# datvo06/MSAU

Measured on AMD Instinct MI355X. Metric: chargrid tiles/sec (train fwd+bwd), 336x256x64 3-stage MSAU, higher is better.
Workload: dtype bf16; 1 GPU; configs[1]: one-hot chargrid 336x256x64, 3-stage MSAU (featRoot 8, 4 scales, res_depth 2), batch 16/GPU, fwd+masked-CE+bwd+clip+Adam; global_batch=16, parallelism=dp1, graph=False

## Files before the change

include/msau_hip.h:

```cpp
#ifndef MSAU_HIP_H
#define MSAU_HIP_H

#include <stdint.h>

#ifdef __cplusplus
extern "C" {
#endif

typedef enum { MSAU_F32 = 0, MSAU_BF16 = 1 } msau_dtype;

typedef enum {
    MSAU_OK = 0,
    MSAU_ERR_ARG = -1,
    MSAU_ERR_LDS = -2,
    MSAU_ERR_HIP = -3
} msau_status;

const char* msau_last_error(void);
int msau_version(void);
const char* msau_source_hash(void);
int msau_sizeof(int which);
int msau_lds_pixel_stride(int raw_bytes, int esz, int c8_per_chunk, int read_stride);
int msau_lds_wrow_stride(int nks, int esz);

enum {
    MSAU_CONV_RELU_IN  = 1,
    MSAU_CONV_RELU_OUT = 2,
    MSAU_CONV_ADD      = 4,
    MSAU_CONV_ACCUM    = 8,
    MSAU_CONV_MASK_A   = 16,
    MSAU_CONV_MASK_B   = 32,
    MSAU_CONV_DOUT     = 128,
    MSAU_CONV_LRN      = 256,
    MSAU_CONV_POOL     = 512,
    MSAU_CONV_IDS      = 1024,
    MSAU_CONV_OWNER    = 2048,
    MSAU_CONV_NCHW     = 4096,
    MSAU_CONV_WGRAD    = 8192,
    MSAU_CONV_ELU      = 32768,
    MSAU_CONV_EXTENT   = 65536,
    MSAU_CONV_HEAD     = 64
};

typedef struct {
    int32_t B, Hin, Win, Hout, Wout;
    int32_t C1, C2;
    int32_t Cout;
    int32_t KH, KW, dil;
    int32_t pad_t, pad_l;
    int32_t stride;
    int32_t ups;
    int32_t flags;
    const void* x1;
    const void* x2;
    const void* wpack;
    const float* bias;
    const void* add;
    const void* mask_a;
    const void* mask_b;
    void* y;
    float* head_probs;
    uint8_t* head_argmax;
    int32_t head_classes;
    int32_t flags2;
    void* y2;
    const void* mask_b2;
    float lrn_alpha_over_n, lrn_beta, lrn_k;
    int32_t reserved0;
    void* pool_y;
    uint8_t* pool_idx;
    const void* wg_x1;
    float* wg_slabs;
    int32_t wg_nslabs;
    int32_t reserved1;
    const int32_t* extent;
} msau_conv_desc;
int msau_conv2d_rider_slabs(int dtype, const msau_conv_desc* d);

typedef struct {
    int32_t cch;
    int32_t nchunks;
    int32_t kchunk;
    int32_t rows;
    int64_t bytes;
} msau_conv_pack_geom;

int msau_conv_pack_geometry(int dtype, int C1_stored, int C2_stored, int Cout_stored, int KH, int KW, int dil,
                            int stride, int ups, msau_conv_pack_geom* out);
int msau_conv2d(void* stream, int dtype, const msau_conv_desc* d);
int msau_conv2d_launch_info(int dtype, const msau_conv_desc* d, int32_t* info8);

enum { MSAU_PAIR_RELU_IN = 1, MSAU_PAIR_RELU_MID = 2, MSAU_PAIR_MASK_MID = 4,
       MSAU_PAIR_LRN_BWD = 16,
       MSAU_PAIR_WGRAD1 = 32,
       MSAU_PAIR_COUPLE = 64,
       MSAU_PAIR_DCOUPLE = 128,
       MSAU_PAIR_TILES = 8 };
typedef struct {
    int32_t B, H, W, C;
    int32_t flags1, flags2;
    const void* x;
    const void* w1;
    const float* b1;
    const void* mask_mid;
    void* mid;
    const void* w2;
    const float* b2;
    const void* add;
    const void* mask_a;
    const void* mask_b;
    void* y;
    void* pool_y;
    uint8_t* pool_idx;
    uint8_t* bits_mid;
    uint8_t* bits_a;
    const void* lrn_a;
    void* lrn_da;
    float lrn_alpha_over_n, lrn_beta, lrn_k;
    int32_t reserved0;
    const void* wg1_x;
    float* wg1_slabs;
    int32_t wg1_nslabs;
    int32_t reserved1;
    const void* cpl_prev;
    const void* cpl_w;
    const float* cpl_b;
    void* cpl_y;
    void* cpl_pool_y;
    uint8_t* cpl_pool_idx;
    const void* dcp_dz;
    const void* dcp_w;
    const void* dcp_mask;
    void* dcp_dprev;
} msau_conv_pair_desc;
int msau_conv_pair_applicable(int dtype, const msau_conv_pair_desc* d);
int msau_conv_pair(void* stream, int dtype, const msau_conv_pair_desc* d);
int64_t msau_conv_pair_bits_bytes(int dtype, const msau_conv_pair_desc* d);
int msau_conv_pair_wgrad_slabs(int dtype, const msau_conv_pair_desc* d);
int msau_conv_pair_instance(int dtype, const msau_conv_pair_desc* d);
void msau_reload_env(void);

typedef struct {
    int32_t B, Hin, Win, Hout, Wout;
    int32_t C1, C2, Cout;
    int32_t KH, KW, dil, pad_t, pad_l, stride;
    int32_t flags;
    const void* x1;
    const void* x2;
    const void* g;
    float* slabs;
    int32_t nslabs;
} msau_wgrad_desc;

typedef struct {
    int32_t cch, nchunks;
    int32_t kext;
    int32_t max_slabs;
    int64_t slab_bytes;
    int32_t lean;
    int32_t reserved;
} msau_wgrad_geom;

int msau_wgrad_geometry(int dtype, const msau_wgrad_desc* d, msau_wgrad_geom* out);
int msau_conv2d_wgrad(void* stream, int dtype, const msau_wgrad_desc* d);
int msau_conv2d_wgrad_groupable(int dtype, const msau_wgrad_desc* a, const msau_wgrad_desc* b);
int msau_conv2d_wgrad_group(void* stream, int dtype, const msau_wgrad_desc* const* ds, int n);

typedef struct {
    int64_t src_off;
    int64_t dst_off;
    int32_t kind;
    int32_t dim0, dim1;
    int32_t KH, KW;
// ... 69 lines not shown
    const void* add;
    const void* mask_b;
    void* dx;
    int64_t npix;
    int32_t C, accumulate;
} msau_attn_proj_bwd_args;
int msau_attn_proj_bwd(void* stream, int dtype, const msau_attn_proj_bwd_args* a);

typedef struct {
    const void* g;
    const void* w1_pack; const void* w2_pack;
    void* dx1; void* dx2;
    const void* mask1; const void* mask2;
    int64_t npix;
    int32_t C, accumulate1, accumulate2, reserved;
} msau_dgrad2_args;
int msau_dgrad2_1x1(void* stream, int dtype, const msau_dgrad2_args* a);

int msau_label_counts(void* stream, const int64_t* labels, int32_t* counts, int B, int64_t hw);
int msau_label_counts_split(void* stream, const int64_t* labels, int32_t* partial, int B, int64_t hw, int K);
int64_t msau_ce_ws_floats(int64_t npix_total);
int msau_masked_ce(void* stream, int dtype, const void* logits, const int64_t* labels, const int32_t* counts,
                   void* dlogits, float* loss_accum, float* ws, int B, int64_t hw, int C, int Cs, float scale);
int64_t msau_ce_multi_ws_floats(int64_t npix_total);
int msau_masked_ce_multi(void* stream, int dtype, const void* logits, const void* aux, const int64_t* labels,
                         const int32_t* counts, void* dlogits, void* daux, float* loss, float* ws,
                         int B, int64_t hw, int C, int Cs, float scale, int counts_k);

int msau_softmax_ce(void* stream, int dtype, const void* logits, const int64_t* labels, void* dlogits,
                    float* loss_accum, float* ws, int B, int64_t hw, int C, int Cs, float scale);
int msau_softmax_ce_weighted(void* stream, int dtype, const void* logits, const int64_t* labels, const float* class_w,
                             void* dlogits, float* sums, float* ws, int B, int64_t hw, int C, int Cs);

int64_t msau_adam_ws_floats(int64_t n);
int msau_clip_adam_step(void* stream, float* params, const float* grads, float* m, float* v, float* state,
                        float* ws, int64_t n, float lr, float beta1, float beta2, float eps, float max_norm,
                        float grad_scale);

int msau_raster_owner(void* stream, const int32_t* boxes, int n, int32_t* owner, int B, int H, int W);
int msau_raster_onehot(void* stream, int dtype, const int32_t* boxes, const int32_t* owner, void* grid_nhwc,
                       int B, int H, int W, int C, int Cs);
int msau_raster_labels(void* stream, const int32_t* boxes, const int32_t* owner, int64_t* labels, int B, int H, int W);
int msau_raster_dense(void* stream, int dtype, const int32_t* boxes, const int32_t* owner, const float* feats,
                      void* grid_nhwc, int B, int H, int W, int C, int Cs);

int64_t msau_box_integral_ws_floats(int B, int H, int W, int C);
int msau_box_integral(void* stream, int dtype, const void* in_nhwc, float* ii, float* ws, int B, int H, int W, int C, int Cs, int relu_in);
int msau_box_params(void* stream, const float* flat_params, int64_t off_hmin, int64_t off_hmax, int64_t off_wmin, int64_t off_wmax,
                    int C, int F, float max_h, float max_w, float* params_fwd, float* params_refl);
int msau_box_filter(void* stream, int dtype, const float* ii, const float* params, void* out_nhwc, int B, int H, int W, int C, int F,
                    int Cs_out, int sum_filters, int accumulate, const void* mask_a, const void* add, const void* mask_b);
int64_t msau_box_pgrad_ws_floats(int B, int H, int W, int C, int F);
int msau_box_param_grad(void* stream, int dtype, const float* ii, const float* params, const void* gout_nhwc, float* ws, float* flat_grads,
                        int64_t off_hmin, int64_t off_hmax, int64_t off_wmin, int64_t off_wmax, int B, int H, int W, int C, int F,
                        int Cs_out, float max_h, float max_w);

typedef struct {
    const void* in; float* ii; const float* params_fwd; const float* params_refl; void* out;
    const void* gout; void* gin; float* ii_g; float* ws; float* flat_grads; float* ws_ii;
    const void* mask_a; const void* add; const void* mask_b;
    int64_t off_hmin, off_hmax, off_wmin, off_wmax;
    int32_t B, H, W, C, F, Cs_in, Cs_out, relu_in, accumulate;
    float max_h, max_w;
} msau_box_args;
int msau_box_fwd(void* stream, int dtype, const msau_box_args* a);
int msau_box_bwd(void* stream, int dtype, const msau_box_args* a);

enum {
    MSAU_OP_CONV2D = 1,
    MSAU_OP_WGRAD = 2,
    MSAU_OP_LRN_FWD = 3,
    MSAU_OP_LRN_BWD = 4,
    MSAU_OP_POOL_FWD = 5,
    MSAU_OP_POOL_BWD = 6,
    MSAU_OP_ATTN_FWD = 7,
    MSAU_OP_ATTN_BWD = 8,
    MSAU_OP_CHANNEL_SUM = 9,
    MSAU_OP_WGRAD_REDUCE = 10,
    MSAU_OP_CONV_PAIR = 11,
    MSAU_OP_BOX_FWD = 12,
    MSAU_OP_BOX_BWD = 13,
    MSAU_OP_ALLREDUCE = 14,
    MSAU_OP_ATTN_PROJ_BWD = 15,
    MSAU_OP_DGRAD2_1X1 = 16
};
typedef struct { int32_t kind; int32_t dtype; const void* args; } msau_op;
typedef struct { const void* a; const void* dy; void* out; int64_t npix; int32_t C, Cs, n; float alpha, beta, k; } msau_lrn_args;
typedef struct { const void* x_or_dy; void* y_or_dx; uint8_t* idx; const void* mask; int32_t B, H, W, Cs, accumulate;
                 const int32_t* extent; } msau_pool_args;
typedef struct { const void* f; const void* g; const void* h; const void* x_or_dy; void* y; float* stats;
                 void* df; void* dg; void* dh; float* ws; int32_t B, N, Ds, Cs; const int32_t* extent; int32_t W, reserved0; } msau_attn_args;
typedef struct { const void* g; int64_t npix; int32_t Cs; float* partials; int32_t nblk; } msau_csum_args;
typedef struct { const float* slab_arena; float* flat_grads; const msau_unpack_entry* table_dev; int32_t n_entries, max_elems; } msau_reduce_args;
typedef struct { void* comm; float* buf; int64_t count; } msau_allreduce_args;
int msau_run_ops(void* stream, const msau_op* ops, int n);
#define MSAU_OP_SIDE 0x100
int msau_run_ops_overlap(void* stream, void* side_stream, const msau_op* ops, int n, int join);
#define MSAU_OP_JOIN 0x800
#define MSAU_OP_PROBE 0x200
#define MSAU_OP_COMM 0x400
int msau_run_ops_dp(void* stream, void* side_stream, void* comm_stream, const msau_op* ops, int n, int join);
int msau_probe_read(float* us, int cap, int* n);
int msau_probe_overhead(void* stream, int reps, float* us);

int msau_comm_available(void);
int msau_comm_unique_id(void* id128_out, int bytes);
int msau_comm_init(void** comm_out, int world, int rank, const void* id128, int bytes);
int msau_comm_destroy(void* comm);
int msau_allreduce_bucket(void* stream, void* comm, float* buf, int64_t count);

typedef struct {
    const int32_t* owner;
    const int32_t* boxes;
    const float* feats;
    const float* w;
    float* wt;
    float* table;
    float* sums;
    float* csum;
    int32_t n_boxes, n_vec, C, csum_blocks;
    int32_t wt_floats;
    int32_t reserved0;
} msau_owner_ctx;

int msau_owner_slabs(const msau_wgrad_desc* d);

int msau_spin(void* stream, int microseconds);
int msau_fill_zero(void* stream, void* p, int64_t bytes);
int msau_fork_visibility_check(void* stream, void* side_stream, int iters, int64_t words, int system_fence, int64_t* mismatches);
int msau_stream_create(int priority, void** stream_out);
int msau_stream_destroy(void* stream);
int msau_softmax_channels_nchw(void* stream, const float* logits, float* pred, int B, int C, int64_t hw);

int msau_softmax_argmax_nhwc(void* stream, int dtype, const void* logits, float* probs, uint8_t* argmax,
                             int64_t npix, int C, int Cs);
int msau_onehot_ids(void* stream, int dtype, const int32_t* ids, void* grid_nhwc, int64_t npix, int C, int Cs);
int msau_onehot_ids_ext(void* stream, int dtype, const int32_t* ids, void* grid_nhwc, int B, int H, int W, int C, int Cs,
                        const int32_t* extent);
int msau_eval_confusion(void* stream, int dtype, const void* logits, const int64_t* labels, int64_t* counts, int B, int H, int W,
                        int C, int Cs, int zero_as, const int32_t* extent);

#ifdef __cplusplus
}
#endif
#endif
```

msau_amd/_lib.py:

```python
from __future__ import annotations

import ctypes as C
import os

HERE = os.path.dirname(os.path.abspath(__file__))
LIB_PATH = os.environ.get("MSAU_HIP_LIB", os.path.join(HERE, "libmsau_hip.so"))

F32, BF16 = 0, 1

CONV_RELU_IN, CONV_RELU_OUT, CONV_ADD, CONV_ACCUM, CONV_MASK_A, CONV_MASK_B, CONV_HEAD, CONV_DOUT = 1, 2, 4, 8, 16, 32, 64, 128
CONV_LRN, CONV_POOL, CONV_IDS, CONV_OWNER, CONV_NCHW, CONV_WGRAD, CONV_ELU = 256, 512, 1024, 2048, 4096, 8192, 32768
CONV_EXTENT = 65536

i32, i64, vp, f32 = C.c_int32, C.c_int64, C.c_void_p, C.c_float


class ConvDesc(C.Structure):
    _fields_ = [(n, i32) for n in ("B", "Hin", "Win", "Hout", "Wout", "C1", "C2", "Cout", "KH", "KW", "dil",
                                   "pad_t", "pad_l", "stride", "ups", "flags")] + \
               [(n, vp) for n in ("x1", "x2", "wpack", "bias", "add", "mask_a", "mask_b", "y", "head_probs", "head_argmax")] + \
               [("head_classes", i32), ("flags2", i32), ("y2", vp), ("mask_b2", vp)] + \
               [("lrn_alpha_over_n", f32), ("lrn_beta", f32), ("lrn_k", f32), ("reserved0", i32), ("pool_y", vp), ("pool_idx", vp)] + \
               [("wg_x1", vp), ("wg_slabs", vp), ("wg_nslabs", i32), ("reserved1", i32), ("extent", vp)]

# ... 10 lines not shown


class BoxArgs(C.Structure):
    _fields_ = [(n, vp) for n in ("in_", "ii", "params_fwd", "params_refl", "out", "gout", "gin", "ii_g", "ws", "flat_grads", "ws_ii",
                                  "mask_a", "add", "mask_b")] + \
               [(n, i64) for n in ("off_hmin", "off_hmax", "off_wmin", "off_wmax")] + \
               [(n, i32) for n in ("B", "H", "W", "C", "F", "Cs_in", "Cs_out", "relu_in", "accumulate")] + \
               [("max_h", f32), ("max_w", f32)]


class ConvPackGeom(C.Structure):
    _fields_ = [("cch", i32), ("nchunks", i32), ("kchunk", i32), ("rows", i32), ("bytes", i64)]


class WgradDesc(C.Structure):
    _fields_ = [(n, i32) for n in ("B", "Hin", "Win", "Hout", "Wout", "C1", "C2", "Cout", "KH", "KW", "dil",
                                   "pad_t", "pad_l", "stride", "flags")] + \
               [(n, vp) for n in ("x1", "x2", "g", "slabs")] + [("nslabs", i32)]


class WgradGeom(C.Structure):
    _fields_ = [("cch", i32), ("nchunks", i32), ("kext", i32), ("max_slabs", i32), ("slab_bytes", i64),
                ("lean", i32), ("reserved", i32)]


class PackEntry(C.Structure):
    _fields_ = [("src_off", i64), ("dst_off", i64)] + \
               [(n, i32) for n in ("kind", "dim0", "dim1", "KH", "KW", "row_is_dim0", "flip", "row_off", "rows_real",
                                   "rows_pad", "k1_real", "k1_store", "k2_real", "k2_store", "cch", "nchunks",
                                   "kchunk", "dtype")]


class UnpackEntry(C.Structure):
    _fields_ = [("slab_off", i64), ("w_off", i64), ("b_off", i64), ("b_src_off", i64), ("b_slab_stride", i64)] + \
               [(n, i32) for n in ("b_elem_stride", "b_nslabs", "b_count", "nslabs", "slab_elems", "kext", "dim0", "dim1", "KH",
                                   "KW", "row_is_dim0", "rows_real", "k1_real", "k1_store", "k2_real", "k2_store",
                                   "cch", "nchunks", "accumulate")]


class Op(C.Structure):
    _fields_ = [("kind", i32), ("dtype", i32), ("args", vp)]


class LrnArgs(C.Structure):
    _fields_ = [("a", vp), ("dy", vp), ("out", vp), ("npix", i64), ("C", i32), ("Cs", i32), ("n", i32),
                ("alpha", f32), ("beta", f32), ("k", f32)]


class PoolArgs(C.Structure):
    _fields_ = [("x_or_dy", vp), ("y_or_dx", vp), ("idx", vp), ("mask", vp)] + \
               [(n, i32) for n in ("B", "H", "W", "Cs", "accumulate")] + [("extent", vp)]


class AttnArgs(C.Structure):
    _fields_ = [(n, vp) for n in ("f", "g", "h", "x_or_dy", "y", "stats", "df", "dg", "dh", "ws")] + \
               [(n, i32) for n in ("B", "N", "Ds", "Cs")] + [("extent", vp), ("W", i32), ("reserved0", i32)]


class CsumArgs(C.Structure):
    _fields_ = [("g", vp), ("npix", i64), ("Cs", i32), ("partials", vp), ("nblk", i32)]


class ReduceArgs(C.Structure):
    _fields_ = [("slab_arena", vp), ("flat_grads", vp), ("table_dev", vp), ("n_entries", i32), ("max_elems", i32)]


class AllreduceArgs(C.Structure):
    _fields_ = [("comm", vp), ("buf", vp), ("count", i64)]


class OwnerCtx(C.Structure):
    _fields_ = [(n, vp) for n in ("owner", "boxes", "feats", "w", "wt", "table", "sums", "csum")] + \
               [(n, i32) for n in ("n_boxes", "n_vec", "C", "csum_blocks", "wt_floats", "reserved0")]


class AttnProjBwdArgs(C.Structure):
    _fields_ = [(n, vp) for n in ("df", "dg", "dh", "wf_pack", "wg_pack", "wh_pack", "add", "mask_b", "dx")] + \
               [("npix", i64), ("C", i32), ("accumulate", i32)]


class Dgrad2Args(C.Structure):
    _fields_ = [(n, vp) for n in ("g", "w1_pack", "w2_pack", "dx1", "dx2", "mask1", "mask2")] + \
               [("npix", i64), ("C", i32), ("accumulate1", i32), ("accumulate2", i32), ("reserved", i32)]


OP_SIDE = 0x100
OP_PROBE = 0x200
OP_COMM = 0x400
OP_JOIN = 0x800
OP_ALLREDUCE = 14
OP_WGRAD_REDUCE = 10
OP_CONV_PAIR = 11
OP_BOX_FWD, OP_BOX_BWD = 12, 13
OP_ATTN_PROJ_BWD = 15
OP_DGRAD2_1X1 = 16
OP_CONV2D, OP_WGRAD, OP_LRN_FWD, OP_LRN_BWD, OP_POOL_FWD, OP_POOL_BWD, OP_ATTN_FWD, OP_ATTN_BWD, OP_CHANNEL_SUM = range(1, 10)

_SIGNATURES = {
    "msau_last_error": (C.c_char_p, []),
    "msau_version": (C.c_int, []),
    "msau_source_hash": (C.c_char_p, []),
    "msau_sizeof": (C.c_int, [C.c_int]),
    "msau_lds_pixel_stride": (C.c_int, [C.c_int, C.c_int, C.c_int, C.c_int]),
    "msau_lds_wrow_stride": (C.c_int, [C.c_int, C.c_int]),
    "msau_conv_pack_geometry": (C.c_int, [C.c_int] * 9 + [C.POINTER(ConvPackGeom)]),
    "msau_conv2d": (C.c_int, [vp, C.c_int, C.POINTER(ConvDesc)]),
    "msau_conv2d_rider_slabs": (C.c_int, [C.c_int, C.POINTER(ConvDesc)]),
    "msau_attn_proj_bwd": (C.c_int, [vp, C.c_int, C.POINTER(AttnProjBwdArgs)]),
    "msau_dgrad2_1x1": (C.c_int, [vp, C.c_int, C.POINTER(Dgrad2Args)]),
    "msau_conv2d_launch_info": (C.c_int, [C.c_int, C.POINTER(ConvDesc), C.POINTER(i32)]),
    "msau_conv_pair_applicable": (C.c_int, [C.c_int, C.POINTER(ConvPairDesc)]),
    "msau_conv_pair": (C.c_int, [vp, C.c_int, C.POINTER(ConvPairDesc)]),
    "msau_conv_pair_bits_bytes": (C.c_int64, [C.c_int, C.POINTER(ConvPairDesc)]),
    "msau_conv_pair_instance": (C.c_int, [C.c_int, C.POINTER(ConvPairDesc)]),
    "msau_conv_pair_wgrad_slabs": (C.c_int, [C.c_int, C.POINTER(ConvPairDesc)]),
    "msau_owner_slabs": (C.c_int, [C.POINTER(WgradDesc)]),
    "msau_comm_available": (C.c_int, []),
    "msau_comm_unique_id": (C.c_int, [vp, C.c_int]),
    "msau_comm_init": (C.c_int, [C.POINTER(vp), C.c_int, C.c_int, vp, C.c_int]),
    "msau_comm_destroy": (C.c_int, [vp]),
    "msau_allreduce_bucket": (C.c_int, [vp, vp, vp, C.c_int64]),
    "msau_run_ops_dp": (C.c_int, [vp, vp, vp, C.POINTER(Op), C.c_int, C.c_int]),
    "msau_reload_env": (None, []),
    "msau_wgrad_geometry": (C.c_int, [C.c_int, C.POINTER(WgradDesc), C.POINTER(WgradGeom)]),
    "msau_conv2d_wgrad": (C.c_int, [vp, C.c_int, C.POINTER(WgradDesc)]),
    "msau_conv2d_wgrad_groupable": (C.c_int, [C.c_int, C.POINTER(WgradDesc), C.POINTER(WgradDesc)]),
    "msau_conv2d_wgrad_group": (C.c_int, [vp, C.c_int, C.POINTER(C.POINTER(WgradDesc)), C.c_int]),
    "msau_pack_params": (C.c_int, [vp, vp, vp, vp, C.c_int, C.c_int]),
    "msau_wgrad_reduce": (C.c_int, [vp, vp, vp, vp, C.c_int, C.c_int]),
    "msau_channel_sum": (C.c_int, [vp, C.c_int, vp, i64, C.c_int, vp, C.c_int]),
    "msau_nchw_to_nhwc": (C.c_int, [vp, C.c_int, vp, vp] + [C.c_int] * 5),
    "msau_nhwc_to_nchw": (C.c_int, [vp, C.c_int, vp, vp] + [C.c_int] * 5),
    "msau_nchw_grad_to_nhwc": (C.c_int, [vp, C.c_int, vp, vp] + [C.c_int] * 6),
    "msau_lrn_fwd": (C.c_int, [vp, C.c_int, vp, vp, i64, C.c_int, C.c_int, C.c_int, f32, f32, f32]),
    "msau_lrn_bwd": (C.c_int, [vp, C.c_int, vp, vp, vp, i64, C.c_int, C.c_int, C.c_int, f32, f32, f32]),
    "msau_maxpool2x2_fwd": (C.c_int, [vp, C.c_int, vp, vp, vp] + [C.c_int] * 4),
    "msau_maxpool2x2_bwd": (C.c_int, [vp, C.c_int, vp, vp, vp, vp] + [C.c_int] * 5),
    "msau_selfattn_fwd": (C.c_int, [vp, C.c_int, vp, vp, vp, vp, vp, vp] + [C.c_int] * 4),
    "msau_selfattn_bwd": (C.c_int, [vp, C.c_int, vp, vp, vp, vp, vp, vp, vp, vp, vp] + [C.c_int] * 4),
    "msau_maxpool2x2_bwd_ext": (C.c_int, [vp, C.c_int, vp, vp, vp, vp] + [C.c_int] * 5 + [vp]),
    "msau_selfattn_fwd_ext": (C.c_int, [vp, C.c_int, vp, vp, vp, vp, vp, vp] + [C.c_int] * 4 + [vp, C.c_int]),
    "msau_selfattn_bwd_ext": (C.c_int, [vp, C.c_int, vp, vp, vp, vp, vp, vp, vp, vp, vp] + [C.c_int] * 4 + [vp, C.c_int]),
    "msau_extent_copy": (C.c_int, [vp, vp, vp] + [C.c_int] * 5 + [vp]),
    "msau_label_counts": (C.c_int, [vp, vp, vp, C.c_int, i64]),
    "msau_label_counts_split": (C.c_int, [vp, vp, vp, C.c_int, i64, C.c_int]),
    "msau_ce_ws_floats": (i64, [i64]),
    "msau_ce_multi_ws_floats": (i64, [i64]),
    "msau_masked_ce_multi": (C.c_int, [vp, C.c_int, vp, vp, vp, vp, vp, vp, vp, vp, C.c_int, i64, C.c_int, C.c_int, f32, C.c_int]),
    "msau_masked_ce": (C.c_int, [vp, C.c_int, vp, vp, vp, vp, vp, vp, C.c_int, i64, C.c_int, C.c_int, f32]),
    "msau_softmax_ce": (C.c_int, [vp, C.c_int, vp, vp, vp, vp, vp, C.c_int, i64, C.c_int, C.c_int, f32]),
    "msau_softmax_ce_weighted": (C.c_int, [vp, C.c_int, vp, vp, vp, vp, vp, vp, C.c_int, i64, C.c_int, C.c_int]),
    "msau_adam_ws_floats": (i64, [i64]),
    "msau_clip_adam_step": (C.c_int, [vp, vp, vp, vp, vp, vp, vp, i64, f32, f32, f32, f32, f32, f32]),
    "msau_raster_owner": (C.c_int, [vp, vp, C.c_int, vp, C.c_int, C.c_int, C.c_int]),
    "msau_raster_onehot": (C.c_int, [vp, C.c_int, vp, vp, vp] + [C.c_int] * 5),
    "msau_raster_labels": (C.c_int, [vp, vp, vp, vp, C.c_int, C.c_int, C.c_int]),
    "msau_raster_dense": (C.c_int, [vp, C.c_int, vp, vp, vp, vp] + [C.c_int] * 5),
    "msau_box_integral_ws_floats": (i64, [C.c_int] * 4),
    "msau_box_integral": (C.c_int, [vp, C.c_int, vp, vp, vp] + [C.c_int] * 6),
    "msau_box_params": (C.c_int, [vp, vp, i64, i64, i64, i64, C.c_int, C.c_int, f32, f32, vp, vp]),
    "msau_box_filter": (C.c_int, [vp, C.c_int, vp, vp, vp] + [C.c_int] * 8 + [vp, vp, vp]),
    "msau_box_fwd": (C.c_int, [vp, C.c_int, C.POINTER(BoxArgs)]),
    "msau_box_bwd": (C.c_int, [vp, C.c_int, C.POINTER(BoxArgs)]),
    "msau_box_pgrad_ws_floats": (i64, [C.c_int] * 5),
    "msau_box_param_grad": (C.c_int, [vp, C.c_int, vp, vp, vp, vp, vp, i64, i64, i64, i64] + [C.c_int] * 6 + [f32, f32]),
    "msau_run_ops": (C.c_int, [vp, C.POINTER(Op), C.c_int]),
    "msau_run_ops_overlap": (C.c_int, [vp, vp, C.POINTER(Op), C.c_int, C.c_int]),
    "msau_spin": (C.c_int, [vp, C.c_int]),
    "msau_fill_zero": (C.c_int, [vp, vp, i64]),
    "msau_fork_visibility_check": (C.c_int, [vp, vp, C.c_int, i64, C.c_int, C.POINTER(i64)]),
    "msau_stream_create": (C.c_int, [C.c_int, C.POINTER(vp)]),
    "msau_stream_destroy": (C.c_int, [vp]),
    "msau_softmax_channels_nchw": (C.c_int, [vp, vp, vp, C.c_int, C.c_int, i64]),
    "msau_probe_read": (C.c_int, [vp, C.c_int, vp]),
    "msau_probe_overhead": (C.c_int, [vp, C.c_int, vp]),
    "msau_softmax_argmax_nhwc": (C.c_int, [vp, C.c_int, vp, vp, vp, i64, C.c_int, C.c_int]),
    "msau_onehot_ids": (C.c_int, [vp, C.c_int, vp, vp, i64, C.c_int, C.c_int]),
    "msau_onehot_ids_ext": (C.c_int, [vp, C.c_int, vp, vp] + [C.c_int] * 5 + [vp]),
    "msau_eval_confusion": (C.c_int, [vp, C.c_int, vp, vp, vp] + [C.c_int] * 6 + [vp]),
}

EXPORTED_SYMBOLS = tuple(_SIGNATURES)

ABI_STRUCTS = (ConvDesc, WgradDesc, PackEntry, UnpackEntry, Op, LrnArgs, PoolArgs, AttnArgs, CsumArgs, ReduceArgs,
               ConvPackGeom, WgradGeom, ConvPairDesc, BoxArgs, AllreduceArgs, OwnerCtx, AttnProjBwdArgs, Dgrad2Args)


class MsauHipError(RuntimeError):
    pass


_lib = None


def load():
    global _lib
    if _lib is not None:
        return _lib
    if not os.path.exists(LIB_PATH):
        raise MsauHipError(f"{LIB_PATH} not found: the MSAU HIP kernels are not built "
                           f"(run `python -m msau_amd.build`); there is no CPU fallback")
    lib = C.CDLL(LIB_PATH)
    for name, (res, args) in _SIGNATURES.items():
        fn = getattr(lib, name)
        fn.restype = res
        fn.argtypes = args
    for which, st in enumerate(ABI_STRUCTS):
        if lib.msau_sizeof(which) != C.sizeof(st):
            raise MsauHipError(f"{LIB_PATH}: sizeof({st.__name__}) is {lib.msau_sizeof(which)} in the library, "
                               f"{C.sizeof(st)} in msau_amd/_lib.py -- rebuild (python -m msau_amd.build)")
    if "MSAU_HIP_LIB" not in os.environ and os.path.isdir(os.path.join(HERE, "csrc")):
        from .build import source_hash
        have, want = lib.msau_source_hash().decode(), source_hash()
        if have != want:
            raise MsauHipError(f"{LIB_PATH} was built from kernel sources {have}, the tree holds {want}: rebuild "
                               f"(python -m msau_amd.build)")
    _lib = lib
    return lib


def check(rc: int, what: str = ""):
    if rc != 0:
        msg = load().msau_last_error().decode("utf-8", "replace")
        raise MsauHipError(f"{what or 'msau call'} failed (status {rc}): {msg}")


class Profiler:

    def __init__(self):
        self.records = []
        self.key = None

    def summary(self):
        import collections
        out = collections.OrderedDict()
        for key, e0, e1 in self.records:
            c, t = out.get(key, (0, 0.0))
            out[key] = (c + 1, t + e0.elapsed_time(e1))
        return out


_profiler = None


def set_profiler(p):
    global _profiler
    _profiler = p


def call(name: str, *args, key=None):
    if _profiler is None:
        check(getattr(load(), name)(*args), name)
        return
    import torch
    e0 = torch.cuda.Event(enable_timing=True)
    e1 = torch.cuda.Event(enable_timing=True)
    e0.record()
    check(getattr(load(), name)(*args), name)
    e1.record()
    _profiler.records.append((key or name, e0, e1))


_side_streams: dict = {}


def concurrent_stream(device=None, index: int = 0):
    import time
    import torch
# ... 31 lines not shown
```

msau_amd/csrc/conv.hip:

```cpp
#include "msau_common.h"

namespace {

struct ConvGeom {
    int esz, taps, cch, nchunks, kchunk, rows, CT, ngroups;
    int nslices;
};

__host__ __device__ inline int pix_stride_bytes(int cch, int esz) {
    int ps = cch * esz;
    if (((ps >> 4) & 1) == 0) ps += 16;
    return ps;
}

struct TileGeom { int TH, TIH, TIW, PS, WS, in_bytes, w_bytes, tab_bytes, total; };

inline bool conv_compact(int KH, int KW, int dil, int stride, int ups) { return stride == 1 && ups == 1 && dil >= 16 && KH * KW > 1; }

inline TileGeom tile_geom(const ConvGeom& g, int PT, int KH, int KW, int dil, int stride, int ups = 1) {
    TileGeom t;
    t.TH = 4 * PT;
    t.TIH = (t.TH - 1) * stride + (KH - 1) * dil + 1;
    t.TIW = 15 * stride + (KW - 1) * dil + 1;
    if (conv_compact(KH, KW, dil, stride, ups)) { t.TIH = KH * KW * t.TH; t.TIW = 16; }
// ... 223 lines not shown
            if (flags & MSAU_CONV_RELU_OUT) {
                if (flags & MSAU_CONV_ELU) {
#pragma unroll
                    for (int j = 0; j < 4; ++j) v[j] = v[j] > 0.f ? v[j] : expm1f(v[j]);
                } else {
#pragma unroll
                    for (int j = 0; j < 4; ++j) v[j] = fmaxf(v[j], 0.f);
                }
            }
            if (flags & MSAU_CONV_MASK_B) {
                V4 m = load4<T>(mask_b + pbase + co);
                if (flags & MSAU_CONV_ELU) {
#pragma unroll
                    for (int j = 0; j < 4; ++j) v[j] = ((float)m[j] > 0.f) ? v[j] : v[j] * ((float)m[j] + 1.f);
                } else {
#pragma unroll
                    for (int j = 0; j < 4; ++j) v[j] = ((float)m[j] > 0.f) ? v[j] : 0.f;
                }
            }
            if (outside) v = f32x4{0.f, 0.f, 0.f, 0.f};
            V4 o;
#pragma unroll
            for (int j = 0; j < 4; ++j) o[j] = (T)v[j];
            store4<T>(y + pbase + co, o);
        }
    }
}

template <typename T, int CT, int PT>
int launch_conv(hipStream_t s, const ConvArgs& a, int nblocks, int nsplit, int lds) {
    static bool attr_set = false;
    if (!attr_set) {
        hipError_t e = hipFuncSetAttribute(reinterpret_cast<const void*>(&conv_kernel<T, CT, PT>),
                                           hipFuncAttributeMaxDynamicSharedMemorySize, MSAU_LDS_LIMIT);
        if (e != hipSuccess) return msau_set_error(MSAU_ERR_HIP, "conv: hipFuncSetAttribute: %s", hipGetErrorString(e));
        attr_set = true;
    }
    hipLaunchKernelGGL((conv_kernel<T, CT, PT>), dim3(nblocks, nsplit), dim3(256), lds, s, a);
    MSAU_CHECK_LAUNCH("conv_kernel");
    return 0;
}

template <typename T, int CT>
int launch_conv_pt(hipStream_t s, const ConvArgs& a, int PT, int nblocks, int nsplit, int lds) {
    switch (PT) {
        case 4: return launch_conv<T, CT, 4>(s, a, nblocks, nsplit, lds);
        case 2: return launch_conv<T, CT, 2>(s, a, nblocks, nsplit, lds);
        default: return launch_conv<T, CT, 1>(s, a, nblocks, nsplit, lds);
    }
}

template <typename T>
int launch_conv_ct(hipStream_t s, const ConvArgs& a, int CT, int PT, int nblocks, int nsplit, int lds) {
    switch (CT) {
        case 1: return launch_conv_pt<T, 1>(s, a, PT, nblocks, nsplit, lds);
        case 2: return launch_conv_pt<T, 2>(s, a, PT, nblocks, nsplit, lds);
        case 4: return launch_conv_pt<T, 4>(s, a, PT, nblocks, nsplit, lds);
        default: return launch_conv_pt<T, 8>(s, a, PT, nblocks, nsplit, lds);
    }
}

}

extern "C" int msau_conv_pack_geometry(int dtype, int C1, int C2, int Cout, int KH, int KW, int dil, int stride, int ups,
                                       msau_conv_pack_geom* out) {
    ConvGeom g;
    int rc = conv_geom(dtype, C1, C2, Cout, KH, KW, dil, stride, ups, &g);
    if (rc) return rc;
    out->cch = g.cch; out->nchunks = g.nchunks; out->kchunk = g.kchunk; out->rows = g.rows * g.nslices;
    out->bytes = (int64_t)g.nslices * g.nchunks * g.rows * g.kchunk * g.esz;
    return 0;
}

static int conv_plan(int dtype, const msau_conv_desc* d, ConvGeom* gout, TileGeom* tout, int* PTout, int64_t* nbout);
int msau_conv_lean_applicable(int dtype, const msau_conv_desc* d, int nchunks, int CT);
int msau_conv_lean_try(hipStream_t s, int dtype, const msau_conv_desc* d, int kchunk, int nchunks, int CT);
int msau_conv_lean_head_capable(int dtype, const msau_conv_desc* d, int nchunks, int CT);
int msau_conv_lean_dout_capable(int dtype, const msau_conv_desc* d, int nchunks, int CT);
int msau_conv_lean_lrn_capable(int dtype, const msau_conv_desc* d, int nchunks, int CT);
int msau_conv_lean_pool_capable(int dtype, const msau_conv_desc* d, int nchunks, int CT);
int msau_conv_lean_ids_capable(int dtype, const msau_conv_desc* d, int nchunks, int CT);
int msau_conv_chunked_try(hipStream_t s, int dtype, const msau_conv_desc* d, int cch, int kchunk, int nchunks, int CT);
int msau_conv_chunked_capable(int dtype, const msau_conv_desc* d, int cch, int nchunks, int CT);
int msau_firstconv_takes(int dtype, const msau_conv_desc* d);
int msau_firstconv_launch(hipStream_t s, int dtype, const msau_conv_desc* d, int real_channels);

static int conv_takes_extent(int dtype, const msau_conv_desc* d, const ConvGeom& g) {
    const int only_others = MSAU_CONV_HEAD | MSAU_CONV_DOUT | MSAU_CONV_LRN | MSAU_CONV_POOL | MSAU_CONV_IDS | MSAU_CONV_OWNER |
                            MSAU_CONV_NCHW | MSAU_CONV_WGRAD;
    if (d->flags & only_others) return 0;
    if (g.nslices == 1 && (msau_rowconv_takes(dtype, d) || msau_conv_chunked_capable(dtype, d, g.cch, g.nchunks, g.CT) ||
                           msau_conv_lean_applicable(dtype, d, g.nchunks, g.CT)))
        return 0;
    return 1;
}

extern "C" int msau_conv2d_launch_info(int dtype, const msau_conv_desc* d, int32_t* info) {
    MSAU_CHECK_ARG(d && info, "conv2d_launch_info: null pointer");
    ConvGeom g; TileGeom t; int PT; int64_t nb;
    int rc = conv_plan(dtype, d, &g, &t, &PT, &nb);
    if (rc) return rc;
    info[0] = g.CT; info[1] = PT; info[2] = t.total; info[3] = (int32_t)nb; info[4] = g.cch; info[5] = g.nchunks;
    info[6] = msau_conv_lean_applicable(dtype, d, g.nchunks, g.CT);
    if (g.nslices == 1 && msau_rowconv_takes(dtype, d)) info[6] = 3;
    if (g.nslices == 1 && !(d->flags & (MSAU_CONV_HEAD | MSAU_CONV_DOUT | MSAU_CONV_LRN | MSAU_CONV_POOL | MSAU_CONV_IDS)) &&
        msau_conv_chunked_capable(dtype, d, g.cch, g.nchunks, g.CT)) info[6] = 2;
    info[7] = msau_conv_lean_head_capable(dtype, d, g.nchunks, g.CT) | (msau_conv_lean_dout_capable(dtype, d, g.nchunks, g.CT) << 1) |
              (((d->flags & MSAU_CONV_DOUT) && g.nslices == 1 && msau_rowconv_takes(dtype, d)) << 1) |
              (msau_conv_lean_lrn_capable(dtype, d, g.nchunks, g.CT) << 2) | (msau_conv_lean_pool_capable(dtype, d, g.nchunks, g.CT) << 3) |
              (msau_conv_lean_ids_capable(dtype, d, g.nchunks, g.CT) << 4);
    {
        msau_conv_desc p = *d;
        p.flags |= MSAU_CONV_OWNER;
        if (msau_ownerconv_takes(dtype, &p)) info[7] |= 32;
    }
    {
        msau_conv_desc p = *d;
        p.flags |= MSAU_CONV_NCHW;
        if (msau_firstconv_takes(dtype, &p)) info[7] |= 64;
    }
    {
        msau_conv_desc p = *d;
        p.flags |= MSAU_CONV_EXTENT;
        if (conv_takes_extent(dtype, &p, g)) info[7] |= 128;
    }
    if (g.nslices == 1 && !(info[7] & 4)) {
        msau_conv_desc p = *d;
        p.flags |= MSAU_CONV_LRN;
        if (!p.y2) p.y2 = p.y;
        if (!(p.lrn_k > 0.f)) p.lrn_k = 1.f;
        if (msau_rowconv_takes(dtype, &p)) info[7] |= 4;
    }
    return 0;
}

static int conv_plan(int dtype, const msau_conv_desc* d, ConvGeom* gout, TileGeom* tout, int* PTout, int64_t* nbout) {
    ConvGeom g;
    int rc = conv_geom(dtype, d->C1, d->C2, d->Cout, d->KH, d->KW, d->dil, d->stride, d->ups, &g);
    if (rc) return rc;
    int PT = 4;
    auto ntiles = [&](int pt) { return (int64_t)d->B * cdiv(d->Hout, 4 * pt) * cdiv(d->Wout, 16); };
    if (ntiles(4) < 512) PT = ntiles(2) >= 384 ? 2 : 1;
    TileGeom t = tile_geom(g, PT, d->KH, d->KW, d->dil, d->stride, d->ups);
    while (t.total > 150 * 1024 && PT > 1) { PT >>= 1; t = tile_geom(g, PT, d->KH, d->KW, d->dil, d->stride, d->ups); }
    if (t.total > 150 * 1024) return msau_set_error(MSAU_ERR_LDS, "conv2d: tile needs %d B of LDS", t.total);
    int64_t nb = ntiles(PT);
    MSAU_CHECK_ARG(nb < (1ll << 31), "conv2d: grid too large");
    *gout = g; *tout = t; *PTout = PT; *nbout = nb;
    return 0;
}

extern "C" int msau_conv2d(void* stream, int dtype, const msau_conv_desc* d) {
    MSAU_CHECK_ARG(d && d->x1 && d->wpack && d->y, "conv2d: null pointer");
    MSAU_CHECK_ARG(d->B > 0 && d->Hin > 0 && d->Win > 0 && d->Hout > 0 && d->Wout > 0, "conv2d: bad dims");
    MSAU_CHECK_ARG(d->C1 % 8 == 0 && d->C2 % 8 == 0 && (d->C2 == 0 || d->x2), "conv2d: bad sources");
    MSAU_CHECK_ARG(!(d->flags & MSAU_CONV_ADD) || d->add, "conv2d: ADD without pointer");
    MSAU_CHECK_ARG(!(d->flags & MSAU_CONV_MASK_A) || d->mask_a, "conv2d: MASK_A without pointer");
    MSAU_CHECK_ARG(!(d->flags & MSAU_CONV_MASK_B) || d->mask_b, "conv2d: MASK_B without pointer");
    if (d->flags & MSAU_CONV_EXTENT) {
        MSAU_CHECK_ARG(d->extent, "conv2d: MSAU_CONV_EXTENT without extent pointer");
        ConvGeom g;
        int rc = conv_geom(dtype, d->C1, d->C2, d->Cout, d->KH, d->KW, d->dil, d->stride, d->ups, &g);
        if (rc) return rc;
        if (!conv_takes_extent(dtype, d, g))
            return msau_set_error(MSAU_ERR_ARG, "conv2d: MSAU_CONV_EXTENT is not implemented for this launch (flags 0x%x; see "
                                  "msau_conv2d_launch_info info[7] & 128): only the generic tile kernel has it", d->flags);
    }
    if (d->flags & MSAU_CONV_WGRAD)
        MSAU_CHECK_ARG(msau_conv2d_rider_slabs(dtype, d) > 0, "conv2d: MSAU_CONV_WGRAD is not implemented for this launch (msau_conv2d_rider_slabs says 0)");
    if (d->flags & MSAU_CONV_OWNER) {
        MSAU_CHECK_ARG(msau_ownerconv_takes(dtype, d), "conv2d: MSAU_CONV_OWNER is the 3x3 stride-1 C -> 8 conv, no other flag but RELU_OUT");
        return msau_ownerconv_fwd(static_cast<hipStream_t>(stream), dtype, d);
    }
    if (d->flags & MSAU_CONV_NCHW) {
        MSAU_CHECK_ARG(msau_firstconv_takes(dtype, d) && d->head_classes > 0 && d->head_classes <= d->C1,
                       "conv2d: MSAU_CONV_NCHW is the bf16 3x3 64 -> 8 conv (W %% 4 == 0, W <= 288), head_classes = real input channels");
        return msau_firstconv_launch(static_cast<hipStream_t>(stream), dtype, d, d->head_classes);
    }
    ConvGeom g; TileGeom t; int PT; int64_t nb;
    int rc = conv_plan(dtype, d, &g, &t, &PT, &nb);
    if (rc) return rc;
    if (d->flags & MSAU_CONV_HEAD) {
        MSAU_CHECK_ARG(d->head_probs && d->head_argmax && d->head_classes > 0 && d->head_classes <= 16 &&
                       d->head_classes <= d->Cout && d->flags == MSAU_CONV_HEAD, "conv2d: bad HEAD arguments");
        if (!msau_conv_lean_head_capable(dtype, d, g.nchunks, g.CT))
            return msau_set_error(MSAU_ERR_ARG, "conv2d: MSAU_CONV_HEAD is not implemented for this launch (see "
                                  "msau_conv2d_launch_info info[7]); run msau_softmax_argmax_nhwc on y instead");
    }
    if (d->flags & MSAU_CONV_DOUT) {
        const int okf = MSAU_CONV_DOUT | MSAU_CONV_ADD | MSAU_CONV_ACCUM | MSAU_CONV_MASK_B | MSAU_CONV_WGRAD;
        MSAU_CHECK_ARG(d->y2 && !(d->flags & ~okf) && !(d->flags2 & ~(MSAU_CONV_ACCUM | MSAU_CONV_MASK_B)) &&
                       (!(d->flags2 & MSAU_CONV_MASK_B) || d->mask_b2), "conv2d: bad DOUT arguments");
        if (!msau_conv_lean_dout_capable(dtype, d, g.nchunks, g.CT) && !(g.nslices == 1 && msau_rowconv_takes(dtype, d)))
            return msau_set_error(MSAU_ERR_ARG, "conv2d: MSAU_CONV_DOUT is not implemented for this launch (see "
                                  "msau_conv2d_launch_info info[7]); issue one launch per output instead");
    }
    if (d->flags & MSAU_CONV_LRN) {
        MSAU_CHECK_ARG(d->y2 && !(d->flags & ~(MSAU_CONV_LRN | MSAU_CONV_RELU_IN)) && d->lrn_k > 0.f, "conv2d: bad LRN arguments");
        if (!msau_conv_lean_lrn_capable(dtype, d, g.nchunks, g.CT) && !(g.nslices == 1 && msau_rowconv_takes(dtype, d)))
            return msau_set_error(MSAU_ERR_ARG, "conv2d: MSAU_CONV_LRN is not implemented for this launch (see "
                                  "msau_conv2d_launch_info info[7]); run msau_lrn_fwd on y instead");
    }
    if (d->flags & MSAU_CONV_IDS) {
        if (!msau_conv_lean_ids_capable(dtype, d, g.nchunks, g.CT))
            return msau_set_error(MSAU_ERR_ARG, "conv2d: MSAU_CONV_IDS is not implemented for this launch (see msau_conv2d_launch_info "
                                  "info[7] & 16); paint the one-hot input with msau_onehot_ids instead");
    }
    if (d->flags & MSAU_CONV_POOL) {
        MSAU_CHECK_ARG(d->pool_y && !(d->flags & (MSAU_CONV_DOUT | MSAU_CONV_HEAD | MSAU_CONV_LRN)), "conv2d: bad POOL arguments");
        if (!msau_conv_lean_pool_capable(dtype, d, g.nchunks, g.CT))
            return msau_set_error(MSAU_ERR_ARG, "conv2d: MSAU_CONV_POOL is not implemented for this launch (see "
                                  "msau_conv2d_launch_info info[7]); run msau_maxpool2x2_fwd on y instead");
    }
    if (g.nslices == 1 && msau_rowconv_takes(dtype, d))
        return msau_rowconv_launch(static_cast<hipStream_t>(stream), dtype, d, g.kchunk, g.rows);
    if (g.nslices == 1 && !(d->flags & (MSAU_CONV_HEAD | MSAU_CONV_DOUT | MSAU_CONV_LRN | MSAU_CONV_POOL | MSAU_CONV_IDS))) {
        rc = msau_conv_chunked_try(static_cast<hipStream_t>(stream), dtype, d, g.cch, g.kchunk, g.nchunks, g.CT);
        if (rc != 0) return rc < 0 ? rc : 0;
    }
    if (g.nslices == 1) {
        rc = msau_conv_lean_try(static_cast<hipStream_t>(stream), dtype, d, g.kchunk, g.nchunks, g.CT);
        if (rc != 0) return rc < 0 ? rc : 0;
    }
    if (d->flags & MSAU_CONV_DOUT) return msau_set_error(MSAU_ERR_ARG, "conv2d: DOUT launch was not taken by a lean instance");
    MSAU_CHECK_ARG(g.nslices == 1 || !(d->flags & MSAU_CONV_HEAD), "conv2d: HEAD with more than 128 output channels");
    hipStream_t s = static_cast<hipStream_t>(stream);
    static const int split_wgs = getenv("MSAU_CONV_ROWSPLIT") ? atoi(getenv("MSAU_CONV_ROWSPLIT")) : 768;
    int cts = g.CT;
    while (cts > 1 && nb * g.nslices * (g.CT / cts) < split_wgs) cts >>= 1;
    const int w_bytes = roundup(cts * 16 * t.WS, 16), lds_total = t.in_bytes + w_bytes + t.tab_bytes;
    for (int sl = 0; sl < g.nslices; ++sl) {
        ConvArgs a;
        a.d = *d;
        a.ystride = d->Cout;
        a.compact = conv_compact(d->KH, d->KW, d->dil, d->stride, d->ups);
        if (g.nslices > 1) {
            const size_t co0 = (size_t)sl * 128, esz = g.esz;
            a.d.Cout = d->Cout - (int)co0 < 128 ? d->Cout - (int)co0 : 128;
            a.d.wpack = static_cast<const char*>(d->wpack) + (size_t)sl * g.nchunks * g.rows * g.kchunk * esz;
            if (d->bias) a.d.bias = d->bias + co0;
            a.d.y = static_cast<char*>(d->y) + co0 * esz;
            if (d->add) a.d.add = static_cast<const char*>(d->add) + co0 * esz;
            if (d->mask_a) a.d.mask_a = static_cast<const char*>(d->mask_a) + co0 * esz;
            if (d->mask_b) a.d.mask_b = static_cast<const char*>(d->mask_b) + co0 * esz;
        }
        a.cch = g.cch; a.nchunks = g.nchunks; a.kchunk = g.kchunk; a.ngroups = g.ngroups;
        a.TIH = t.TIH; a.TIW = t.TIW; a.PS = t.PS; a.WS = t.WS; a.in_bytes = t.in_bytes; a.w_bytes = w_bytes;
        a.tiles_x = cdiv(d->Wout, 16); a.tiles_y = cdiv(d->Hout, 4 * PT);
        a.ct_total = g.CT; a.rows_total = g.rows;
        rc = dtype == MSAU_F32 ? launch_conv_ct<float>(s, a, cts, PT, (int)nb, g.CT / cts, lds_total)
                               : launch_conv_ct<bf16_t>(s, a, cts, PT, (int)nb, g.CT / cts, lds_total);
        if (rc) return rc;
    }
    return 0;
}
```

msau_amd/csrc/conv_lean.hip:

```cpp
#include "msau_common.h"
#include <cstdlib>

namespace {

struct LeanArgs {
    msau_conv_desc d;
    int kchunk;
    int in_px1, in_px2, in_row1, in_row2;
    int out_px, out_row;
    int tiles_x, tiles_y, ntiles;
    unsigned mag_tx, mag_ty;
    int per_xcd;
    int ct_total;
#ifdef MSAU_STAMPS
    unsigned long long* stamps;
#endif
};
#ifdef MSAU_STAMPS
#define STAMP(i) do { if (a.stamps && threadIdx.x == 0) a.stamps[((size_t)blockIdx.y * gridDim.x + blockIdx.x) * 8 + (i)] = __builtin_amdgcn_s_memrealtime(); } while (0)
#else
#define STAMP(i) do {} while (0)
#endif

template <typename T, int CIN8, int CT, int KS, bool DUAL, int DIL = 1, int WGW = 1, int STRIDE = 1>
struct LeanCfg {
    static constexpr int ESZ = (int)sizeof(T);
    static constexpr int TI = 15 * STRIDE + 1 + (KS - 1) * DIL;
    static constexpr int TIW = (16 * WGW - 1) * STRIDE + 1 + (KS - 1) * DIL;
    static constexpr int NT = 256 * WGW;
    static constexpr int PSRAW = CIN8 * 8 * ESZ;
    static constexpr int NPIX = TI * TIW;
    static constexpr int NCH = DUAL ? 2 : 1;
    static constexpr int C8H = CIN8 / NCH;
    static constexpr int PS = lds_pixel_stride(PSRAW, ESZ, C8H, STRIDE);
    static constexpr int NG = KS * KS * C8H;
    static constexpr int NKSH = (NG + 3) / 4;
    static constexpr int NKS = NCH * NKSH;
    static constexpr bool WREG = CT * NKS <= 8;
    static constexpr int WS = lds_wrow_stride(NKSH, ESZ);
    static constexpr int IN_BYTES = ((NPIX * PS + 15) / 16) * 16;
    static constexpr int LDS = IN_BYTES + (WREG ? 0 : NCH * CT * 16 * WS);
};

constexpr int kOperandBits = MSAU_CONV_RELU_IN | MSAU_CONV_RELU_OUT | MSAU_CONV_ADD | MSAU_CONV_ACCUM | MSAU_CONV_MASK_A | MSAU_CONV_MASK_B;
enum { EPI_NONE = 0, EPI_LRN = 1, EPI_POOL = 2, EPI_HEAD = 3 };
template <typename T, int CIN8, int CT, int KS, bool DUAL, int DIL = 1, int WGW = 1, bool DOUT = false, bool SPLIT = false,
          int STRIDE = 1, int UPS = 1, int EPI = EPI_NONE, int EOP = -1, bool IDS = false>
__global__ __launch_bounds__(256 * WGW) void conv_lean_kernel(const LeanArgs a) {
    static_assert(!IDS || (!DUAL && STRIDE == 1 && UPS == 1 && !DOUT && !SPLIT), "id-mask input: plain single-source instances");
    static_assert(!SPLIT || (CT == 1 && !DUAL && !DOUT && WGW == 1), "SPLIT instances are single-source, one tile per workgroup");
    static_assert((STRIDE == 1 && UPS == 1) || (!DUAL && !DOUT && WGW == 1 && DIL == 1 && STRIDE * UPS == 2), "strided / upsampling instances");
    STAMP(0);
    const int cty = SPLIT ? (int)blockIdx.y : 0;
    const int CTT = SPLIT ? a.ct_total : CT;
    using Cfg = LeanCfg<T, CIN8, CT, KS, DUAL, DIL, WGW, STRIDE>;
    constexpr int NT = Cfg::NT;
    typedef typename Vec8<T>::type V8;
    typedef typename Vec4<T>::type V4;
    constexpr int ESZ = Cfg::ESZ, TI = Cfg::TIW, PS = Cfg::PS, NKS = Cfg::NKS, NG = Cfg::NG, NKSH = Cfg::NKSH, C8H = Cfg::C8H;
    extern __shared__ __align__(16) unsigned char smem[];
    const msau_conv_desc& d = a.d;
    const int tid = threadIdx.x, lane = tid & 63;
    const int wave_all = __builtin_amdgcn_readfirstlane(tid >> 6);
    const int wave = wave_all & 3, cwt = wave_all >> 2;
    const int lr = lane & 15, lg = lane >> 4;
    const bool relu_in = (EOP >= 0 ? EOP : d.flags) & MSAU_CONV_RELU_IN;

    const T* wp = static_cast<const T*>(d.wpack) + (SPLIT ? (size_t)cty * 16 * a.kchunk : 0);
    V8 afr[Cfg::WREG ? CT : 1][Cfg::WREG ? NKS : 1];
    if constexpr (Cfg::WREG) {
#pragma unroll
        for (int ct = 0; ct < CT; ++ct)
#pragma unroll
            for (int ks = 0; ks < NKS; ++ks)
                afr[ct][ks] = load8<T>(wp + ((size_t)(ks / NKSH) * (CT * 16) + ct * 16 + lr) * a.kchunk + (ks % NKSH) * 32 + lg * 8);
    }

    int koff[NKS];
#pragma unroll
    for (int ks = 0; ks < NKS; ++ks) {
        const int G = (ks % NKSH) * 4 + lg;
        const int tap = G / C8H, cg = G - tap * C8H;
        const int ky = tap / KS, kx = tap - ky * KS;
        koff[ks] = G < NG ? (ky * DIL * TI + kx * DIL) * PS + ((ks / NKSH) * C8H + cg) * 8 * ESZ : 0;
    }
    const unsigned char* pixp = smem + ((wave * 4) * STRIDE * TI + (cwt * 16 + lr) * STRIDE) * PS;

    const int flags = EOP >= 0 ? ((d.flags & ~kOperandBits) | EOP) : d.flags;
    const int Cout = d.Cout;
    f32x4 bv[CT];
#pragma unroll
    for (int ct = 0; ct < CT; ++ct) {
        bv[ct] = f32x4{0.f, 0.f, 0.f, 0.f};
        if (d.bias && lg * (CTT * 4) + (cty + ct) * 4 < Cout) bv[ct] = *reinterpret_cast<const f32x4*>(d.bias + lg * (CTT * 4) + (cty + ct) * 4);
    }
    const long long delta_add = static_cast<const char*>(d.add) - static_cast<const char*>(d.y);
    const long long delta_ma = static_cast<const char*>(d.mask_a) - static_cast<const char*>(d.y);
    const long long delta_mb = static_cast<const char*>(d.mask_b) - static_cast<const char*>(d.y);
    const int lane_out = (cwt * 16 + lr) * a.out_px + (lg * (CTT * 4) + cty * 4) * ESZ;

    constexpr int C8S = DUAL ? CIN8 / 2 : CIN8;
    constexpr int NITEMS = Cfg::NPIX * C8S;
    constexpr int NIT = (NITEMS + NT - 1) / NT;
    constexpr int NSRC = DUAL ? 2 : 1;
    constexpr bool PIPE = IDS || NIT * NSRC <= 6;
    V8 pre[IDS ? 1 : NSRC][IDS ? 1 : NIT];
    constexpr int NIDS = (Cfg::NPIX + NT - 1) / NT;
    int pre_id[IDS ? NIDS : 1];
    auto decode = [&](int tile, int& b, int& oy0, int& ox0) {
        const int t1 = a.tiles_x > 1 ? __umulhi((unsigned)tile, a.mag_tx) : tile;
        ox0 = (tile - t1 * a.tiles_x) * (16 * WGW);
        b = a.tiles_y > 1 ? __umulhi((unsigned)t1, a.mag_ty) : t1;
        oy0 = (t1 - b * a.tiles_y) * 16;
    };
    auto issue_loads = [&](int tile) {
        int b, oy0, ox0;
        decode(tile, b, oy0, ox0);
        const int vy0 = oy0 * STRIDE - d.pad_t, vx0 = ox0 * STRIDE - d.pad_l;
        if constexpr (IDS) {
            const int* ids = static_cast<const int*>(d.x1) + (long long)b * d.Hin * d.Win;
#pragma unroll
            for (int it = 0; it < NIDS; ++it) {
                const int pix = tid + it * NT;
                const int iy = pix / TI, ix = pix - iy * TI;
                const int vy = vy0 + iy, vx = vx0 + ix;
                pre_id[it] = -1;
                if (pix < Cfg::NPIX && (unsigned)vy < (unsigned)d.Hin && (unsigned)vx < (unsigned)d.Win) pre_id[it] = ids[vy * d.Win + vx];
            }
        } else
#pragma unroll
        for (int sidx = 0; sidx < NSRC; ++sidx) {
// ... 85 lines not shown
    }

    STAMP(1);
    for (int tile = tile0; tile < tend; tile += tstep) {
        int b, oy0, ox0;
        decode(tile, b, oy0, ox0);
        __syncthreads();
        if (!PIPE) issue_loads(tile);
        write_lds();
        __syncthreads();
        if (tile == tile0) STAMP(2);
        if (PIPE && tile + tstep < tend) issue_loads(tile + tstep);
        const int oyw = oy0 + wave * 4;
        f32x4 acc[CT][4];
#pragma unroll
        for (int ct = 0; ct < CT; ++ct)
#pragma unroll
            for (int pt = 0; pt < 4; ++pt) acc[ct][pt] = f32x4{0.f, 0.f, 0.f, 0.f};
#pragma unroll
        for (int ks = 0; ks < NKS; ++ks) {
            const unsigned char* p = pixp + koff[ks];
            V8 bfrag[4];
#pragma unroll
            for (int pt = 0; pt < 4; ++pt) bfrag[pt] = *reinterpret_cast<const V8*>(p + pt * STRIDE * TI * PS);
#pragma unroll
            for (int ct = 0; ct < CT; ++ct) {
                V8 af;
                if constexpr (Cfg::WREG) af = afr[ct][ks];
                else af = *reinterpret_cast<const V8*>(smem + Cfg::IN_BYTES + ((ks / NKSH) * (CT * 16) + ct * 16 + lr) * Cfg::WS +
                                                       ((ks % NKSH) * 32 + lg * 8) * ESZ);
#pragma unroll
                for (int pt = 0; pt < 4; ++pt) acc[ct][pt] = mma8(af, bfrag[pt], acc[ct][pt]);
            }
        }

        if (tile == tile0) { asm volatile("" :: "v"(acc[0][0][0])); STAMP(3); }
        if constexpr (DOUT) {
            const bool t2 = lg >= 2;
            const int lfl = t2 ? d.flags2 : flags;
            char* yb = static_cast<char*>(t2 ? d.y2 : d.y);
            const char* mb = static_cast<const char*>(t2 ? d.mask_b2 : d.mask_b);
            const char* ad = static_cast<const char*>(d.add);
            if (ox0 + lr < d.Wout) {
                const long long off0 = ((long long)(b * d.Hout + oyw)) * a.out_row + (long long)ox0 * a.out_px +
                                       lr * a.out_px + (lg & 1) * (CT * 4) * ESZ;
#pragma unroll
                for (int ct = 0; ct < CT; ++ct) {
                    V4 r_add[4], r_acc[4], r_mb[4];
#pragma unroll
                    for (int pt = 0; pt < 4; ++pt) {
                        if (oyw + pt < d.Hout) {
                            const long long o = off0 + ct * 4 * ESZ + (long long)pt * a.out_row;
                            if (lfl & MSAU_CONV_ADD) r_add[pt] = *reinterpret_cast<const V4*>(ad + o);
                            if (lfl & MSAU_CONV_ACCUM) r_acc[pt] = *reinterpret_cast<const V4*>(yb + o);
                            if (lfl & MSAU_CONV_MASK_B) r_mb[pt] = *reinterpret_cast<const V4*>(mb + o);
                        }
                    }
#pragma unroll
                    for (int pt = 0; pt < 4; ++pt) {
                        if (oyw + pt < d.Hout) {
                            const long long o = off0 + ct * 4 * ESZ + (long long)pt * a.out_row;
                            f32x4 v = acc[ct][pt] + bv[ct];
                            if (lfl & MSAU_CONV_ADD) {
#pragma unroll
                                for (int j = 0; j < 4; ++j) v[j] += (float)r_add[pt][j];
                            }
                            if (lfl & MSAU_CONV_ACCUM) {
#pragma unroll
                                for (int j = 0; j < 4; ++j) v[j] += (float)r_acc[pt][j];
                            }
                            if (lfl & MSAU_CONV_MASK_B) {
#pragma unroll
                                for (int j = 0; j < 4; ++j) v[j] = ((float)r_mb[pt][j] > 0.f) ? v[j] : 0.f;
                            }
                            V4 ov;
#pragma unroll
                            for (int j = 0; j < 4; ++j) ov[j] = (T)v[j];
                            *reinterpret_cast<V4*>(yb + o) = ov;
                        }
                    }
                }
            }
        } else {
        constexpr bool POOL_OK = EPI == EPI_POOL;
        static_assert(EPI == EPI_NONE || (CT <= 2 && !DOUT && STRIDE == 1 && UPS == 1), "fused epilogues: <= 2 channel tiles, one output");
        V4 keep[POOL_OK ? CT : 1][4];
        if constexpr (POOL_OK) {
#pragma unroll
            for (int ct = 0; ct < CT; ++ct)
#pragma unroll
                for (int pt = 0; pt < 4; ++pt)
#pragma unroll
                    for (int j = 0; j < 4; ++j) keep[ct][pt][j] = (T)0.f;
        }
        if (ox0 + cwt * 16 + lr < d.Wout) {
            char* y = static_cast<char*>(d.y) + ((long long)(b * d.Hout + oyw)) * a.out_row + (long long)ox0 * a.out_px;
#pragma unroll
            for (int ct = 0; ct < CT; ++ct) {
                if (lg * (CTT * 4) + (cty + ct) * 4 >= Cout) continue;
#pragma unroll
                for (int pt = 0; pt < 4; ++pt) {
                    if (oyw + pt < d.Hout) {
                        char* yp = y + (unsigned)(lane_out + ct * 4 * ESZ + pt * a.out_row);
                        f32x4 v = acc[ct][pt] + bv[ct];
                        if (flags & (MSAU_CONV_MASK_A | MSAU_CONV_ADD | MSAU_CONV_ACCUM | MSAU_CONV_RELU_OUT | MSAU_CONV_MASK_B)) {
                            if (flags & MSAU_CONV_MASK_A) {
                                V4 m = *reinterpret_cast<const V4*>(yp + delta_ma);
#pragma unroll
                                for (int j = 0; j < 4; ++j) v[j] = ((float)m[j] > 0.f) ? v[j] : 0.f;
                            }
                            if (flags & MSAU_CONV_ADD) {
                                V4 r = *reinterpret_cast<const V4*>(yp + delta_add);
#pragma unroll
                                for (int j = 0; j < 4; ++j) v[j] += (float)r[j];
                            }
                            if (flags & MSAU_CONV_ACCUM) {
                                V4 r = *reinterpret_cast<const V4*>(yp);
#pragma unroll
                                for (int j = 0; j < 4; ++j) v[j] += (float)r[j];
                            }
                            if (flags & MSAU_CONV_RELU_OUT) {
#pragma unroll
                                for (int j = 0; j < 4; ++j) v[j] = fmaxf(v[j], 0.f);
                            }
                            if (flags & MSAU_CONV_MASK_B) {
                                V4 m = *reinterpret_cast<const V4*>(yp + delta_mb);
#pragma unroll
                                for (int j = 0; j < 4; ++j) v[j] = ((float)m[j] > 0.f) ? v[j] : 0.f;
                            }
                        }
                        V4 o;
#pragma unroll
                        for (int j = 0; j < 4; ++j) o[j] = (T)v[j];
                        *reinterpret_cast<V4*>(yp) = o;
                        if constexpr (POOL_OK) keep[ct][pt] = o;
                    }
                }
            }
        }
        if constexpr (POOL_OK) {
            if (flags & MSAU_CONV_POOL) {
                const int Ho = (d.Hout + 1) >> 1, Wo = (d.Wout + 1) >> 1;
                const int col = ox0 + cwt * 16 + lr;
                constexpr int ND = (int)sizeof(V4) / 4;
#pragma unroll
                for (int ct = 0; ct < CT; ++ct) {
#pragma unroll
                    for (int pp = 0; pp < 2; ++pp) {
                        V4 nb[2];
#pragma unroll
                        for (int r = 0; r < 2; ++r) {
                            typedef int dwords __attribute__((ext_vector_type(ND)));
                            dwords src = __builtin_bit_cast(dwords, keep[ct][2 * pp + r]), dst;
#pragma unroll
                            for (int w = 0; w < ND; ++w) dst[w] = __builtin_amdgcn_mov_dpp(src[w], 0xB1, 0xf, 0xf, true);
                            nb[r] = __builtin_bit_cast(V4, dst);
                        }
                        const int r0 = oyw + 2 * pp;
                        if (!(lr & 1) && r0 < d.Hout && col < d.Wout && lg * (CTT * 4) + (cty + ct) * 4 < Cout) {
                            V4 best;
                            unsigned idx = 0;
#pragma unroll
                            for (int j = 0; j < 4; ++j) {
                                float bv_ = (float)keep[ct][2 * pp][j];
                                unsigned bi = 0;
                                const float c1 = (float)nb[0][j], c2 = (float)keep[ct][2 * pp + 1][j], c3 = (float)nb[1][j];
                                if (c1 > bv_) { bv_ = c1; bi = 1; }
                                if (c2 > bv_) { bv_ = c2; bi = 2; }
                                if (c3 > bv_) { bv_ = c3; bi = 3; }
                                best[j] = (T)bv_;
                                idx |= bi << (8 * j);
                            }
                            const long long e = (((long long)b * Ho + (r0 >> 1)) * Wo + (col >> 1)) * Cout + lg * (CTT * 4) + (cty + ct) * 4;
                            *reinterpret_cast<V4*>(static_cast<T*>(d.pool_y) + e) = best;
                            if (d.pool_idx) *reinterpret_cast<unsigned*>(d.pool_idx + e) = idx;
                        }
                    }
                }
            }
        }
        }
        if constexpr (EPI == EPI_LRN) {
            static_assert(!SPLIT && !DUAL, "LRN needs all channels of a pixel in one workgroup");
            if (flags & MSAU_CONV_LRN) {
                const int RL = Cout == 8 ? 2 : 4;
                const bool b075 = d.lrn_beta == 0.75f;
                char* y2 = static_cast<char*>(d.y2) + ((long long)(b * d.Hout + oyw)) * a.out_row + (long long)ox0 * a.out_px;
#pragma unroll
                for (int pt = 0; pt < 4; ++pt) {
                    float x[CT * 4], P[CT * 4];
                    float run = 0.f;
#pragma unroll
                    for (int ct = 0; ct < CT; ++ct) {
                        const f32x4 v = acc[ct][pt] + bv[ct];
#pragma unroll
                        for (int j = 0; j < 4; ++j) {
                            const float r = (float)(T)v[j];
                            x[ct * 4 + j] = r;
                            run += r * r;
                            P[ct * 4 + j] = run;
                        }
                    }
                    float inc = run;
                    const float n1 = __shfl(inc, lane - 16);
                    if (lg >= 1) inc += n1;
                    const float n2 = __shfl(inc, lane - 32);
                    if (lg >= 2) inc += n2;
                    const float E = inc - run;
                    const float tot = __shfl(inc, lr + 16 * (RL - 1));
                    V4 o[CT];
#pragma unroll
                    for (int i = 0; i < CT * 4; ++i) {
                        const float X = E + (i ? P[i - 1] : 0.f);
                        const float Xo = __shfl(X, lane ^ (8 * RL));
                        const float win = lg < RL / 2 ? Xo : tot - Xo;
                        const float dd = d.lrn_k + d.lrn_alpha_over_n * win;
                        float dnb;
                        if (b075) { const float r = __builtin_amdgcn_rsqf(dd); dnb = r * __builtin_amdgcn_sqrtf(r); }
                        else dnb = __expf(-d.lrn_beta * __logf(dd));
// ... 444 lines not shown
        attr_set = true;
    }
    int per_cu = MSAU_LDS_LIMIT / (lds + 256);
    per_cu = per_cu < 1 ? 1 : (per_cu > 3 ? 3 : per_cu);
    int grid = 256 * per_cu;
    if (grid > a.ntiles) grid = a.ntiles;
    hipLaunchKernelGGL((conv_chunked_kernel<T, C8CH, CT, DIL>), dim3(grid), dim3(256), lds, s, a, nchunks);
    MSAU_CHECK_LAUNCH("conv_chunked_kernel");
    return 1;
}

int msau_conv_chunked_try(hipStream_t s, int dtype, const msau_conv_desc* d, int cch, int kchunk, int nchunks, int CT) {
    const int variant = chunked_variant(dtype, d, cch, nchunks, CT);
    if (!variant) return 0;
    const int esz = dtype == MSAU_F32 ? 4 : 2;
    LeanArgs a;
    a.d = *d;
    a.kchunk = kchunk;
    a.in_px1 = d->C1 * esz; a.in_row1 = d->Win * a.in_px1; a.in_px2 = a.in_row2 = 0;
    a.out_px = d->Cout * esz; a.out_row = d->Wout * a.out_px;
    a.tiles_x = cdiv(d->Wout, 16); a.tiles_y = cdiv(d->Hout, 16);
    a.ntiles = d->B * a.tiles_x * a.tiles_y;
    a.mag_tx = (unsigned)((0x100000000ull + a.tiles_x - 1) / a.tiles_x);
    a.mag_ty = (unsigned)((0x100000000ull + a.tiles_y - 1) / a.tiles_y);
    a.per_xcd = 0; a.ct_total = CT;
#ifdef MSAU_STAMPS
    a.stamps = nullptr;
#endif
    if (variant == 2) return launch_chunked<bf16_t, 4, 2, 8>(s, a, nchunks);
    return dtype == MSAU_F32 ? launch_chunked<float, 8, 1, 1>(s, a, nchunks) : launch_chunked<bf16_t, 8, 1, 1>(s, a, nchunks);
}

int msau_conv_lean_try(hipStream_t s, int dtype, const msau_conv_desc* d, int kchunk, int nchunks, int CT) {
    if (!msau_conv_lean_applicable(dtype, d, nchunks, CT)) return 0;
    const bool dual = d->C2 != 0;
    const int cin8 = (d->C1 + d->C2) / 8;
    const int esz = dtype == MSAU_F32 ? 4 : 2;
    LeanArgs a;
    a.d = *d;
    a.kchunk = kchunk;
    a.in_px1 = d->C1 * esz; a.in_px2 = d->C2 * esz;
    a.in_row1 = d->Win * a.in_px1; a.in_row2 = d->Win * a.in_px2;
    const bool dout = d->flags & MSAU_CONV_DOUT;
    a.out_px = (dout ? d->Cout / 2 : d->Cout) * esz; a.out_row = d->Wout * a.out_px;
    a.tiles_x = cdiv(d->Wout, 16); a.tiles_y = cdiv(d->Hout, 16);
    a.ntiles = d->B * a.tiles_x * a.tiles_y;
    if (a.ntiles >= (1 << 20) || a.tiles_x >= 4096 || a.tiles_y >= 4096) return 0;
    a.mag_tx = (unsigned)((0x100000000ull + a.tiles_x - 1) / a.tiles_x);
    a.mag_ty = (unsigned)((0x100000000ull + a.tiles_y - 1) / a.tiles_y);
    a.ct_total = CT;
#ifdef MSAU_STAMPS
    a.stamps = std::getenv("MSAU_STAMP_PTR") ? reinterpret_cast<unsigned long long*>(strtoull(std::getenv("MSAU_STAMP_PTR"), nullptr, 0)) : nullptr;
#endif
    if (d->stride * d->ups == 2)
        return dtype == MSAU_F32 ? lean_strided<float>(s, a, cin8, CT, d->ups == 2) : lean_strided<bf16_t>(s, a, cin8, CT, d->ups == 2);
    if (d->flags & MSAU_CONV_IDS) {
        if (!msau_conv_lean_ids_capable(dtype, d, nchunks, CT)) return 0;
        return dtype == MSAU_F32 ? launch_lean_e<float, 8, 1, 3, false, 1, 1, false, false, 1, 1, EPI_NONE, -1, true>(s, a)
                                 : launch_lean_e<bf16_t, 8, 1, 3, false, 1, 1, false, false, 1, 1, EPI_NONE, -1, true>(s, a);
    }
    if (d->flags & MSAU_CONV_HEAD) {
        if (!msau_conv_lean_head_capable(dtype, d, nchunks, CT)) return 0;
        return dtype == MSAU_F32 ? launch_lean<float, 1, 1, 4, false, 1, 1, false, false, 1, 1, EPI_HEAD>(s, a)
                                 : launch_lean<bf16_t, 1, 1, 4, false, 1, 1, false, false, 1, 1, EPI_HEAD>(s, a);
    }
    if (d->flags & (MSAU_CONV_LRN | MSAU_CONV_POOL)) {
        const int which = lean_epi_case(dtype, d, CT, (d->flags & MSAU_CONV_LRN) ? EPI_LRN : EPI_POOL);
        if (!which) return msau_set_error(MSAU_ERR_ARG, "conv_lean: no instance with this fused epilogue (msau_conv2d_launch_info)");
        return dtype == MSAU_F32 ? lean_epi<float>(s, a, which) : lean_epi<bf16_t>(s, a, which);
    }
    if (lean_split_wanted(d, CT))
        return dtype == MSAU_F32 ? lean_split<float>(s, a, cin8, d->KH) : lean_split<bf16_t>(s, a, cin8, d->KH);
    if (dout) {
        if (!msau_conv_lean_dout_capable(dtype, d, nchunks, CT)) return 0;
        return dtype == MSAU_F32 ? lean_dout<float>(s, a, d->KH, CT) : lean_dout<bf16_t>(s, a, d->KH, CT);
    }
    if (d->dil == 2) return dtype == MSAU_F32 ? lean_dil<float, 2>(s, a, cin8, CT) : lean_dil<bf16_t, 2>(s, a, cin8, CT);
    if (d->dil == 4) return dtype == MSAU_F32 ? lean_dil<float, 4>(s, a, cin8, CT) : lean_dil<bf16_t, 4>(s, a, cin8, CT);
    if (d->dil == 8) return dtype == MSAU_F32 ? lean_dil<float, 8>(s, a, cin8, CT) : lean_dil<bf16_t, 8>(s, a, cin8, CT);
    if (d->KH == 4) return dtype == MSAU_F32 ? lean_ct<float, 1, 4, false>(s, a, CT) : lean_ct<bf16_t, 1, 4, false>(s, a, CT);
    if (dtype == MSAU_F32) return d->KH == 3 ? lean_cin<float, 3>(s, a, cin8, dual, CT) : lean_cin<float, 1>(s, a, cin8, dual, CT);
    return d->KH == 3 ? lean_cin<bf16_t, 3>(s, a, cin8, dual, CT) : lean_cin<bf16_t, 1>(s, a, cin8, dual, CT);
}
```

msau_amd/csrc/pack.hip:

```cpp
#include "msau_common.h"
#include <cstdlib>

static thread_local char g_err[512] = "";

int msau_set_error(int code, const char* fmt, ...) {
    va_list ap;
    va_start(ap, fmt);
    vsnprintf(g_err, sizeof(g_err), fmt, ap);
    va_end(ap);
    return code;
}

extern "C" const char* msau_last_error(void) { return g_err; }
extern "C" int msau_version(void) { return 11; }

extern "C" int msau_lds_pixel_stride(int raw_bytes, int esz, int c8_per_chunk, int read_stride) { return lds_pixel_stride(raw_bytes, esz, c8_per_chunk, read_stride); }
extern "C" int msau_lds_wrow_stride(int nks, int esz) { return lds_wrow_stride(nks, esz); }

extern "C" int msau_sizeof(int which) {
    switch (which) {
        case 0: return (int)sizeof(msau_conv_desc);
        case 1: return (int)sizeof(msau_wgrad_desc);
        case 2: return (int)sizeof(msau_pack_entry);
        case 3: return (int)sizeof(msau_unpack_entry);
        case 4: return (int)sizeof(msau_op);
        case 5: return (int)sizeof(msau_lrn_args);
        case 6: return (int)sizeof(msau_pool_args);
        case 7: return (int)sizeof(msau_attn_args);
        case 8: return (int)sizeof(msau_csum_args);
        case 9: return (int)sizeof(msau_reduce_args);
        case 10: return (int)sizeof(msau_conv_pack_geom);
        case 11: return (int)sizeof(msau_wgrad_geom);
        case 12: return (int)sizeof(msau_conv_pair_desc);
        case 13: return (int)sizeof(msau_box_args);
        case 14: return (int)sizeof(msau_allreduce_args);
        case 15: return (int)sizeof(msau_owner_ctx);
        case 16: return (int)sizeof(msau_attn_proj_bwd_args);
        case 17: return (int)sizeof(msau_dgrad2_args);
        default: return -1;
    }
}

namespace {

__device__ __forceinline__ int real_channel(int cs, int k1_real, int k1_store, int k2_real, int k2_store) {
    if (cs < k1_store) return cs < k1_real ? cs : -1;
    int c2 = cs - k1_store;
    return c2 < k2_real ? k1_real + c2 : -1;
}

__global__ void pack_kernel(const float* __restrict__ params, unsigned char* __restrict__ arena,
                            const msau_pack_entry* __restrict__ table) {
    const msau_pack_entry e = table[blockIdx.y];
    const float* src = params + e.src_off;
    if (e.kind == 1) {
        float* dst = reinterpret_cast<float*>(arena + e.dst_off);
        for (int i = blockIdx.x * blockDim.x + threadIdx.x; i < e.rows_pad; i += gridDim.x * blockDim.x)
            dst[i] = i < e.rows_real ? src[e.row_off + i] : 0.f;
        return;
    }
    const int taps = e.KH * e.KW;
    const int srows = e.rows_pad > 128 ? 128 : e.rows_pad;
    const int CT = srows >> 4;
    const int64_t total = (int64_t)e.nchunks * e.rows_pad * e.kchunk;
    for (int64_t i8 = ((int64_t)blockIdx.x * blockDim.x + threadIdx.x) * 8; i8 < total; i8 += (int64_t)gridDim.x * blockDim.x * 8) {
        const int k0 = (int)(i8 % e.kchunk);
        const int64_t r = i8 / e.kchunk;
        const int slot = (int)(r % srows);
        const int chunk = (int)((r / srows) % e.nchunks);
        const int slice = (int)(r / ((int64_t)srows * e.nchunks));
        const int ct = slot >> 4, q = (slot >> 2) & 3, j = slot & 3;
        const int row = slice * 128 + q * (CT * 4) + ct * 4 + j;
        float v[8];
#pragma unroll
        for (int u = 0; u < 8; ++u) {
            const int k = k0 + u;
            v[u] = 0.f;
            if (row < e.rows_real && k < taps * e.cch) {
                int tap = k / e.cch, c = k - tap * e.cch;
                int kc = real_channel(chunk * e.cch + c, e.k1_real, e.k1_store, e.k2_real, e.k2_store);
                if (kc >= 0) {
                    int ky = tap / e.KW, kx = tap - ky * e.KW;
                    if (e.flip) { ky = e.KH - 1 - ky; kx = e.KW - 1 - kx; }
                    int prow = e.row_off + row;
                    int i0 = e.row_is_dim0 ? prow : kc;
                    int i1 = e.row_is_dim0 ? kc : prow;
                    v[u] = src[(((int64_t)i0 * e.dim1 + i1) * e.KH + ky) * e.KW + kx];
                }
            }
        }
        if (e.dtype == MSAU_F32) {
            float* dst = reinterpret_cast<float*>(arena + e.dst_off) + i8;
            *reinterpret_cast<f32x4*>(dst) = f32x4{v[0], v[1], v[2], v[3]};
            *reinterpret_cast<f32x4*>(dst + 4) = f32x4{v[4], v[5], v[6], v[7]};
        } else {
            bf16x8 o;
#pragma unroll
            for (int u = 0; u < 8; ++u) o[u] = (bf16_t)v[u];
            *reinterpret_cast<bf16x8*>(reinterpret_cast<bf16_t*>(arena + e.dst_off) + i8) = o;
        }
    }
}

__global__ __launch_bounds__(256) void unpack_kernel(const float* __restrict__ slabs, float* __restrict__ grads,
                                                     const msau_unpack_entry* __restrict__ table) {
    constexpr int NC = 64, NS = 16;
    __shared__ float red[NS][NC + 4];
    const msau_unpack_entry e = table[blockIdx.y];
    const int taps = e.KH * e.KW;
    const int kreal = taps * e.cch;
    const int rows_store = e.slab_elems / (e.kext * e.nchunks);
    const int ngroups = (e.slab_elems + NC - 1) / NC;
    const float* s0 = slabs + e.slab_off;
    const int cl = threadIdx.x & 15, sl = threadIdx.x >> 4;
    const bool conv_bias = e.b_off >= 0 && e.b_elem_stride == e.kext;
    for (int grp = blockIdx.x; grp < ngroups; grp += gridDim.x) {
        const int f0 = grp * NC + cl * 4;
        f32x4 a0 = {0.f, 0.f, 0.f, 0.f}, a1 = a0, a2 = a0, a3 = a0;
        if (f0 < e.slab_elems) {
            const float* p = s0 + f0;
            int s = sl;
// ... 97 lines not shown
```

msau_amd/csrc/sequence.hip:

```cpp
#include "msau_common.h"

#include <cstdlib>
#include <utility>
#include <vector>

static int run_one_raw(void* stream, const msau_op& o, int i);

namespace {
struct ProbePair { hipEvent_t a, b; };
thread_local std::vector<ProbePair> g_probe_pool;
thread_local size_t g_probe_used = 0;
}

static int run_one(void* stream, const msau_op& o_in, int i) {
    if (!(o_in.kind & MSAU_OP_PROBE)) return run_one_raw(stream, o_in, i);
    msau_op o = o_in;
    o.kind &= ~MSAU_OP_PROBE;
    if (g_probe_used == g_probe_pool.size()) {
        ProbePair p;
        if (hipEventCreate(&p.a) != hipSuccess || hipEventCreate(&p.b) != hipSuccess)
            return msau_set_error(MSAU_ERR_HIP, "run_ops: cannot create probe events");
        g_probe_pool.push_back(p);
    }
    ProbePair& p = g_probe_pool[g_probe_used++];
// ... 108 lines not shown
            rc = run_one(side_stream, o, pending[i].second);
            if (rc) return rc;
        }
        pending.clear();
        any_side = true;
        return 0;
    };
    auto join_side = [&]() -> int {
        hipEvent_t ev;
        int rc = next_event_of(&ev, true);
        if (rc) return rc;
        if (hipEventRecord(ev, ss) != hipSuccess || hipStreamWaitEvent(ms, ev, 0) != hipSuccess)
            return msau_set_error(MSAU_ERR_HIP, "run_ops_overlap: join failed");
        return 0;
    };
    hipStream_t cs = static_cast<hipStream_t>(comm_stream);
    bool any_comm = false;
    for (int i = 0; i < n; ++i) {
        msau_op o = ops[i];
        const bool side = o.kind & MSAU_OP_SIDE;
        const bool join_first = o.kind & MSAU_OP_JOIN;
        const bool comm = o.kind & MSAU_OP_COMM;
        o.kind &= ~(MSAU_OP_SIDE | MSAU_OP_JOIN | MSAU_OP_COMM);
        if (comm) {
            if (!cs) return msau_set_error(MSAU_ERR_ARG, "run_ops_dp: op %d needs the comm stream", i);
            int rc = flush();
            if (rc) return rc;
            hipEvent_t ev;
            rc = next_event_of(&ev, true);
            if (rc) return rc;
            if (hipEventRecord(ev, any_side ? ss : ms) != hipSuccess || hipStreamWaitEvent(cs, ev, 0) != hipSuccess)
                return msau_set_error(MSAU_ERR_HIP, "run_ops_dp: comm fork failed");
            rc = run_one(comm_stream, o, i);
            if (rc) return rc;
            any_comm = true;
            continue;
        }
        if (side) {
            pending.emplace_back(o, i);
            if ((int)pending.size() >= fork_every || (o.kind & 0xff) == MSAU_OP_WGRAD_REDUCE || (o.kind & 0xff) == MSAU_OP_ATTN_FWD) {
                int rc = flush();
                if (rc) return rc;
            }
            continue;
        }
        if (join_first) {
            int rc = flush();
            if (rc) return rc;
            if (any_side) { rc = join_side(); if (rc) return rc; }
        }
        if ((o.kind & 0xff) == MSAU_OP_WGRAD && !pending.empty()) {
            int rc = flush();
            if (rc) return rc;
        }
        int rc = run_one(stream, o, i);
        if (rc) return rc;
    }
    {
        int rc = flush();
        if (rc) return rc;
    }
    if (any_comm && join) {
        hipEvent_t ev;
        int rc = next_event_of(&ev, true);
        if (rc) return rc;
        if (hipEventRecord(ev, cs) != hipSuccess || hipStreamWaitEvent(ms, ev, 0) != hipSuccess)
            return msau_set_error(MSAU_ERR_HIP, "run_ops_dp: comm join failed");
    }
    if (any_side && join) return join_side();
    return 0;
}

static int run_one_raw(void* stream, const msau_op& o, int i) {
    {
        int rc;
        switch (o.kind) {
            case MSAU_OP_CONV2D: rc = msau_conv2d(stream, o.dtype, static_cast<const msau_conv_desc*>(o.args)); break;
            case MSAU_OP_WGRAD: rc = msau_conv2d_wgrad(stream, o.dtype, static_cast<const msau_wgrad_desc*>(o.args)); break;
            case MSAU_OP_CONV_PAIR: rc = msau_conv_pair(stream, o.dtype, static_cast<const msau_conv_pair_desc*>(o.args)); break;
            case MSAU_OP_BOX_FWD: rc = msau_box_fwd(stream, o.dtype, static_cast<const msau_box_args*>(o.args)); break;
            case MSAU_OP_BOX_BWD: rc = msau_box_bwd(stream, o.dtype, static_cast<const msau_box_args*>(o.args)); break;
            case MSAU_OP_ATTN_PROJ_BWD: rc = msau_attn_proj_bwd(stream, o.dtype, static_cast<const msau_attn_proj_bwd_args*>(o.args)); break;
            case MSAU_OP_DGRAD2_1X1: rc = msau_dgrad2_1x1(stream, o.dtype, static_cast<const msau_dgrad2_args*>(o.args)); break;
            case MSAU_OP_LRN_FWD: {
                const msau_lrn_args* a = static_cast<const msau_lrn_args*>(o.args);
                rc = msau_lrn_fwd(stream, o.dtype, a->a, a->out, a->npix, a->C, a->Cs, a->n, a->alpha, a->beta, a->k);
                break;
            }
            case MSAU_OP_LRN_BWD: {
                const msau_lrn_args* a = static_cast<const msau_lrn_args*>(o.args);
                rc = msau_lrn_bwd(stream, o.dtype, a->a, a->dy, a->out, a->npix, a->C, a->Cs, a->n, a->alpha, a->beta, a->k);
                break;
            }
            case MSAU_OP_POOL_FWD: {
                const msau_pool_args* a = static_cast<const msau_pool_args*>(o.args);
                rc = msau_maxpool2x2_fwd(stream, o.dtype, a->x_or_dy, a->y_or_dx, a->idx, a->B, a->H, a->W, a->Cs);
                break;
            }
            case MSAU_OP_POOL_BWD: {
                const msau_pool_args* a = static_cast<const msau_pool_args*>(o.args);
                rc = msau_maxpool2x2_bwd_ext(stream, o.dtype, a->x_or_dy, a->idx, a->y_or_dx, a->mask, a->B, a->H, a->W, a->Cs, a->accumulate,
                                             a->extent);
                break;
            }
            case MSAU_OP_ATTN_FWD: {
                const msau_attn_args* a = static_cast<const msau_attn_args*>(o.args);
                rc = msau_selfattn_fwd_ext(stream, o.dtype, a->f, a->g, a->h, a->x_or_dy, a->y, a->stats, a->B, a->N, a->Ds, a->Cs,
                                           a->extent, a->W);
                break;
            }
            case MSAU_OP_ATTN_BWD: {
                const msau_attn_args* a = static_cast<const msau_attn_args*>(o.args);
                rc = msau_selfattn_bwd_ext(stream, o.dtype, a->f, a->g, a->h, a->x_or_dy, a->stats, a->df, a->dg, a->dh, a->ws,
                                           a->B, a->N, a->Ds, a->Cs, a->extent, a->W);
                break;
            }
            case MSAU_OP_CHANNEL_SUM: {
                const msau_csum_args* a = static_cast<const msau_csum_args*>(o.args);
                rc = msau_channel_sum(stream, o.dtype, a->g, a->npix, a->Cs, a->partials, a->nblk);
                break;
            }
            case MSAU_OP_WGRAD_REDUCE: {
                const msau_reduce_args* a = static_cast<const msau_reduce_args*>(o.args);
                rc = msau_wgrad_reduce(stream, a->slab_arena, a->flat_grads, a->table_dev, a->n_entries, a->max_elems);
                break;
            }
            case MSAU_OP_ALLREDUCE: {
                const msau_allreduce_args* a = static_cast<const msau_allreduce_args*>(o.args);
                rc = msau_allreduce_bucket(stream, a->comm, a->buf, a->count);
                break;
            }
            default: return msau_set_error(MSAU_ERR_ARG, "run_ops: op %d has unknown kind %d", i, o.kind);
        }
        return rc;
    }
}
```

msau_amd/plan.py:

```python
from __future__ import annotations

import ctypes as C
import math
import os
from typing import Dict, List, Optional, Tuple

import torch

from . import _lib as L


def same_pads(in_size: int, k: int, stride: int = 1, dilation: int = 1) -> Tuple[int, int]:
    k_eff = k + (k - 1) * (dilation - 1)
    out = -(-in_size // stride)
    pad = max((out - 1) * stride + k_eff - in_size, 0)
    return pad // 2, pad - pad // 2


def _ru(a: int, b: int) -> int:
    return -(-a // b) * b


def _ptr(t: Optional[torch.Tensor]) -> Optional[int]:
    return None if t is None else t.data_ptr()
# ... 8 lines not shown
        self.relu_out = relu_out
        self.needs_grad = needs_grad and plan.training
        self.data = None if plan.reuse else torch.zeros((plan.B, H, W, self.Cs), dtype=plan.tdtype, device=plan.device)
        self.grad: Optional[torch.Tensor] = None
        self.n_contrib = 0
        plan.acts.append(self)

    @property
    def npix(self) -> int:
        return self.plan.B * self.H * self.W

    def register(self) -> int:
        k = self.n_contrib
        self.n_contrib += 1
        return k

    def slot_flags(self, k: int) -> Tuple[bool, bool]:
        return k != self.n_contrib - 1, (k == 0 and self.relu_out)

    def alloc_grad(self):
        if self.needs_grad and self.n_contrib > 0 and self.grad is None:
            self.grad = torch.zeros_like(self.data)


class Op:
    name = "op"

    def reads(self) -> List["Act"]:
        return []

    def writes(self) -> List["Act"]:
        return []

    def finalize(self):
        pass

    def note(self):
        pass

    def fwd(self, s):
        raise NotImplementedError

    def bwd(self, s):
        pass


class ConvOp(Op):

    def __init__(self, plan: "Plan", name: str, x1: Act, x2: Optional[Act], wname: str, bname: str, out: Act,
                 k: int, dil: int = 1, relu_in: bool = False, relu_out: bool = False,
                 fwd_add: Optional[Act] = None, kind: str = "conv", head: bool = False):
        self.plan, self.name, self.x1, self.x2, self.out = plan, name, x1, x2, out
        self.head = head
        self.wname, self.bname, self.k, self.dil, self.kind = wname, bname, k, dil, kind
        self.relu_in, self.relu_out, self.fwd_add = relu_in, relu_out, fwd_add
        self.bwd_add: Optional[Act] = None
        self.pair: Optional["PairOp"] = None
        self.cpl: Optional["ConvOp"] = None
        self.cpl_fused_into: Optional["PairOp"] = None
        self.proj: Optional["ProjBwd"] = None
        self.dgrad2 = None
        self.dgrad_in_pair: Optional["PairOp"] = None
        if kind == "conv" and k == 1 and x2 is not None and relu_out and not relu_in and fwd_add is None and plan.ops:
            prod = plan.ops[-1]
            if isinstance(prod, ConvOp) and prod.out is x2 and prod.pair is not None and prod is prod.pair.c2 \
                    and x1.Cs == x2.Cs == out.Cs == x2.C == out.C:
                prod.cpl = self
        assert out.relu_out == relu_out
        if kind == "conv":
            assert out.H == x1.H and out.W == x1.W
            self.pad_t = same_pads(x1.H, k, 1, dil)[0]
            self.pad_l = same_pads(x1.W, k, 1, dil)[0]
        else:
            assert x2 is None and dil == 1 and not relu_in
            p = k // 2
            for o, i in ((out.H, x1.H), (out.W, x1.W)):
                op = o - ((i - 1) * 2 - 2 * p + k)
                assert 0 <= op < 2, f"{name}: output size {o} unreachable from {i}"
            self.pad_t = self.pad_l = k - 1 - p
        self.slots = []
        for x in (x1, x2):
            self.slots.append(x.register() if (x is not None and x.needs_grad) else None)
        self.stage = plan._cur_stage
        plan.ops.append(self)

    def reduce_group(self):
        return -1 if (self.stage == 0 and self.name.startswith("s0.d0.")) else self.stage

    def reads(self):
        return [t for t in (self.x1, self.x2, self.fwd_add) if t is not None]

    def writes(self):
        lrn, pool = getattr(self, "lrn", None), getattr(self, "pool", None)
        w = [self.out] + ([lrn.y] if lrn is not None else []) + ([pool.y] if pool is not None else [])
        if self.cpl is not None:
            w += [t for t in self.cpl.writes() if t not in w]
        return w

    def _geom(self, C1, C2, Cout, dil, stride, ups):
        g = L.ConvPackGeom()
        L.call("msau_conv_pack_geometry", self.plan.dtype, C1, C2, Cout, self.k, self.k, dil, stride, ups, C.byref(g))
        return g

    def _pack_entry(self, g, off, row_is_dim0, flip, row_off, rows_real, k1, k2):
        shp = self.plan.pshape[self.wname]
        e = L.PackEntry()
        e.src_off = self.plan.poff[self.wname]
        e.dst_off = off
        e.kind, e.dim0, e.dim1, e.KH, e.KW = 0, shp[0], shp[1], self.k, self.k
        e.row_is_dim0, e.flip, e.row_off, e.rows_real, e.rows_pad = int(row_is_dim0), int(flip), row_off, rows_real, g.rows
        e.k1_real, e.k1_store = k1
        e.k2_real, e.k2_store = k2
        e.cch, e.nchunks, e.kchunk, e.dtype = g.cch, g.nchunks, g.kchunk, self.plan.dtype
        return e, g.nchunks * g.rows * g.kchunk

    def finalize(self):
        P = self.plan
        x1, x2, out = self.x1, self.x2, self.out
        C2s = x2.Cs if x2 is not None else 0
        C2r = x2.C if x2 is not None else 0
        conv = self.kind == "conv"
        g = self._geom(x1.Cs, C2s, out.Cs, self.dil, 1, 1 if conv else 2)
        self.w_off = P.alloc_pack(g.bytes)
        e, n = self._pack_entry(g, self.w_off, row_is_dim0=conv, flip=not conv, row_off=0, rows_real=out.C,
                                k1=(x1.C, x1.Cs), k2=(C2r, C2s))
        P.add_pack_entry(e, n)
        self.b_off = P.alloc_pack(out.Cs * 4)
        be = L.PackEntry()
        be.src_off, be.dst_off, be.kind = P.poff[self.bname], self.b_off, 1
        be.row_off, be.rows_real, be.rows_pad = 0, out.C, out.Cs
        P.add_pack_entry(be, out.Cs)
        self.d_off = [None, None]
        self.wg_fused = False
        self.uentry = None
        self.dd_off = None
        if P.training and conv and x2 is not None and None not in self.slots and x1.C == x1.Cs == x2.C == x2.Cs \
                and x1.Cs + x2.Cs <= 128 and os.environ.get("MSAU_FUSE_DGRAD", "1") != "0" and not P.generic_only:
            proto = L.ConvDesc()
            proto.B, proto.Hin, proto.Win, proto.Hout, proto.Wout = P.B, out.H, out.W, x1.H, x1.W
            proto.C1, proto.C2, proto.Cout = out.Cs, 0, x1.Cs + x2.Cs
            proto.KH = proto.KW = self.k
            proto.dil, proto.stride, proto.ups = self.dil, 1, 1
            proto.pad_t = (self.k - 1) * self.dil - self.pad_t
            proto.pad_l = (self.k - 1) * self.dil - self.pad_l
            info = (L.i32 * 8)()
            L.call("msau_conv2d_launch_info", P.dtype, C.byref(proto), info)
            if info[7] & 2:
                gd = self._geom(out.Cs, 0, x1.Cs + x2.Cs, self.dil, 1, 1)
                self.dd_off = P.alloc_pack(gd.bytes)
                e, n = self._pack_entry(gd, self.dd_off, row_is_dim0=False, flip=True, row_off=0,
                                        rows_real=x1.C + x2.C, k1=(out.C, out.Cs), k2=(0, 0))
                P.add_pack_entry(e, n)
        self.dcp_off = self.dd_off
        if P.training and conv and self.k == 1 and x2 is not None and self.dd_off is None and None not in self.slots \
                and x1.C == x1.Cs == x2.C == x2.Cs == out.Cs == 32 and P.dtype == L.BF16 and not P.generic_only \
                and any(pr.c2.cpl is self for pr in P.pairs):
            gd = self._geom(out.Cs, 0, x1.Cs + x2.Cs, self.dil, 1, 1)
            self.dcp_off = P.alloc_pack(gd.bytes)
            e, n = self._pack_entry(gd, self.dcp_off, row_is_dim0=False, flip=True, row_off=0,
                                    rows_real=x1.C + x2.C, k1=(out.C, out.Cs), k2=(0, 0))
            P.add_pack_entry(e, n)
        if P.training and self.dd_off is None:
            for si, x in enumerate((x1, x2)):
                if x is None or self.slots[si] is None:
                    continue
                if conv:
# ... 105 lines not shown
            if maskb:
                fl |= L.CONV_MASK_B | P.act_flag
                dd.mask_b = _ptr(x.data)
            dd.flags = fl | P.extent_flag
            dd.extent = P.extent_ptr(x)
            dd.x1, dd.wpack, dd.bias, dd.y = _ptr(out.grad), P.pack_ptr(self.d_off[si]), None, _ptr(x.grad)
            self.ddesc[si] = dd
        self.dgrad2 = None
        d1, d2 = self.ddesc
        if conv and self.k == 1 and x2 is not None and self.dd_off is None and d1 is not None and d2 is not None \
                and P.dtype == L.BF16 and not P.generic_only and x1.C == x1.Cs == x2.C == x2.Cs == out.Cs == 64 \
                and not ((d1.flags | d2.flags) & ~(L.CONV_ACCUM | L.CONV_MASK_B)) and os.environ.get("MSAU_DGRAD2", "1") != "0":
            geo = [self._geom(out.Cs, 0, x.Cs, 1, 1, 1) for x in (x1, x2)]
            if all((gq.nchunks, gq.rows, gq.kchunk) == (1, 64, 64) for gq in geo):
                a = L.Dgrad2Args()
                a.g, a.w1_pack, a.w2_pack = _ptr(out.grad), P.pack_ptr(self.d_off[0]), P.pack_ptr(self.d_off[1])
                a.dx1, a.dx2 = _ptr(x1.grad), _ptr(x2.grad)
                a.mask1 = d1.mask_b if d1.flags & L.CONV_MASK_B else None
                a.mask2 = d2.mask_b if d2.flags & L.CONV_MASK_B else None
                a.npix, a.C = out.npix, 64
                a.accumulate1, a.accumulate2 = int(bool(d1.flags & L.CONV_ACCUM)), int(bool(d2.flags & L.CONV_ACCUM))
                self.dgrad2 = a
        w = L.WgradDesc()
        w.B = P.B
        w.KH = w.KW = self.k
        if conv:
            w.Hin, w.Win, w.Hout, w.Wout = x1.H, x1.W, out.H, out.W
            w.C1, w.C2, w.Cout = x1.Cs, (x2.Cs if x2 is not None else 0), out.Cs
            w.dil, w.pad_t, w.pad_l, w.stride = self.dil, self.pad_t, self.pad_l, 1
            w.flags = L.CONV_RELU_IN if self.relu_in else 0
            w.x1, w.x2, w.g = _ptr(x1.data), _ptr(x2.data if x2 is not None else None), _ptr(out.grad)
            rows_real, k1, k2 = out.C, (x1.C, x1.Cs), ((x2.C, x2.Cs) if x2 is not None else (0, 0))
        else:
            w.Hin, w.Win, w.Hout, w.Wout = out.H, out.W, x1.H, x1.W
            w.C1, w.C2, w.Cout = out.Cs, 0, x1.Cs
            w.dil, w.pad_t, w.pad_l, w.stride = 1, self.k // 2, self.k // 2, 2
            w.flags = 0
            w.x1, w.x2, w.g = _ptr(out.grad), None, _ptr(x1.data)
            rows_real, k1, k2 = x1.C, (out.C, out.Cs), (0, 0)
        wg = L.WgradGeom()
        w.nslabs = 1
        L.call("msau_wgrad_geometry", P.dtype, C.byref(w), C.byref(wg))
        nslabs = max(1, min(wg.max_slabs, int(os.environ.get('MSAU_SLAB_CAP', '384')), max(int(os.environ.get('MSAU_SLAB_MIN', '64')), (int(os.environ.get('MSAU_SLAB_MB', '3')) << 20) // max(wg.slab_bytes, 1))))
        w.nslabs = nslabs
        slab_elems = wg.slab_bytes // 4
        self.slab_off = P.alloc_slab(nslabs * slab_elems)
        self.wdesc, self.wgeom = w, wg
        shp = P.pshape[self.wname]
        taps = self.k * self.k
        u = L.UnpackEntry()
        u.slab_off, u.w_off, u.b_off = self.slab_off, P.poff[self.wname], P.poff[self.bname]
        u.nslabs, u.slab_elems, u.kext = nslabs, slab_elems, wg.kext
        u.dim0, u.dim1, u.KH, u.KW, u.row_is_dim0, u.rows_real = shp[0], shp[1], self.k, self.k, 1, rows_real
        u.k1_real, u.k1_store = k1
        u.k2_real, u.k2_store = k2
        u.cch, u.nchunks, u.accumulate = wg.cch, wg.nchunks, 0
        if conv:
            u.b_src_off, u.b_slab_stride, u.b_elem_stride, u.b_nslabs = self.slab_off + taps * wg.cch, slab_elems, wg.kext, nslabs
            u.b_count = out.C
        else:
            self.csum_blocks = max(1, min(256, out.npix // 1024))
            self.csum_off = P.alloc_slab(self.csum_blocks * out.Cs)
            u.b_src_off, u.b_slab_stride, u.b_elem_stride, u.b_nslabs = self.csum_off, out.Cs, 1, self.csum_blocks
            u.b_count = out.C
        P.add_unpack_entry(u, slab_elems, self.reduce_group())
        self.uentry = u
        dd = self.ddesc[0]
        if conv and self.k == 1 and x2 is not None and self.dd_off is not None and dd is not None and not self.relu_in \
                and dd.flags == L.CONV_DOUT and dd.flags2 == L.CONV_MASK_B and u.kext == 16 and u.slab_elems == 256 and u.cch == 8 \
                and u.nchunks == 2 and os.environ.get("MSAU_COUPLE_WGRAD", "1") != "0" and P.cfg.get("couple_wgrad", True):
            dd.flags |= L.CONV_WGRAD
            dd.wg_x1, dd.wg_slabs = _ptr(x1.data), 1
            ns = int(L.load().msau_conv2d_rider_slabs(P.dtype, C.byref(dd)))
            if ns > 0:
                dd.wg_nslabs = ns
                self.wg_slab_off = P.alloc_slab(ns * 256)
                u.slab_off, u.nslabs = self.wg_slab_off, ns
                u.b_src_off, u.b_nslabs = self.wg_slab_off + 8, ns
                self.wg_fused = True
            else:
                dd.flags &= ~L.CONV_WGRAD
                dd.wg_x1 = dd.wg_slabs = None

    def late_bind(self):
        P = self.plan
        if self.wdesc is not None:
            self.wdesc.slabs = P.slab_ptr(self.slab_off)
        if self.wg_fused and self.pair is None and self.ddesc[0] is not None and self.ddesc[0].flags & L.CONV_WGRAD:
            self.ddesc[0].wg_slabs = P.slab_ptr(self.wg_slab_off)
        T = "f32" if P.dtype == L.F32 else "bf16"
        esz = 4 if P.dtype == L.F32 else 2
        taps = self.k * self.k
        cin_real = self.x1.C + (self.x2.C if self.x2 is not None else 0)
        self.flops = 2.0 * P.B * (self.out.H * self.out.W if self.kind == "conv" else self.x1.H * self.x1.W) * \
            taps * cin_real * self.out.C

        def conv_meta(d):
            info = (L.i32 * 8)()
            L.call("msau_conv2d_launch_info", P.dtype, C.byref(d), info)
            nin = d.B * d.Hin * d.Win * (d.C1 + d.C2)
            nout = d.B * d.Hout * d.Wout * d.Cout
            extra = sum(1 for f in (L.CONV_ADD, L.CONV_ACCUM, L.CONV_MASK_A, L.CONV_MASK_B, L.CONV_LRN) if d.flags & f)
            if d.flags & L.CONV_DOUT:
                half = nout // 2
                ex1 = sum(1 for f in (L.CONV_ADD, L.CONV_ACCUM, L.CONV_MASK_B) if d.flags & f)
                ex2 = sum(1 for f in (L.CONV_ACCUM, L.CONV_MASK_B) if d.flags2 & f)
                rider = (half * esz + d.wg_nslabs * 256 * 4) if d.flags & L.CONV_WGRAD else 0
                return f"conv_lean_kernel<{T},CIN{d.C1},CT{info[0]},K{d.KH},dout{',wgrad' if rider else ''}>", (nin + half * (2 + ex1 + ex2)) * esz + rider
            if info[6] == 3:
                name = f"rowconv_kernel<{T},CIN{d.C1 + d.C2},CO{d.Cout},K{d.KH}{',lrn' if d.flags & L.CONV_LRN else ''}{',ups2' if d.ups == 2 else ''}>"
            elif info[6] == 2:
                name = f"conv_chunked_kernel<{T},CIN{d.C1},K{d.KH}>"
            elif info[6]:
                var = ",dual" if d.C2 else ",ups2" if d.ups == 2 else ",s2" if d.stride == 2 else ""
                var += ",lrn" if d.flags & L.CONV_LRN else ""
                name = f"conv_lean_kernel<{T},CIN{d.C1 + d.C2},CT{info[0]},K{d.KH}{var}>"
            else:
                name = f"conv_kernel<{T},CT{info[0]},PT{info[1]}>"
            pooled = (nout // 4) * (esz + 1) if d.flags & L.CONV_POOL else 0
            return name, (nin + nout * (1 + extra)) * esz + pooled

        self.fkey, self.fbytes = conv_meta(self.fdesc)
        P.note_launch(self.fkey, self.fbytes, self.flops)
        self.dmeta = [None, None]
        for si, dd in enumerate(self.ddesc):
            if dd is not None:
                src_c = (self.x1.C + self.x2.C) if self.dd_off is not None else (self.x1, self.x2)[si].C
                fl = 2.0 * P.B * (self.out.H * self.out.W if self.kind == "conv" else self.x1.H * self.x1.W) * taps * src_c * self.out.C
                self.dmeta[si] = conv_meta(dd)
                if (self.proj is None or not self.proj.active) and self.dgrad2 is None and self.dgrad_in_pair is None:
                    P.note_launch(self.dmeta[si][0], self.dmeta[si][1], fl)
        if self.dgrad2 is not None:
            a = self.dgrad2
            nops = 3 + a.accumulate1 + a.accumulate2 + (1 if a.mask1 else 0) + (1 if a.mask2 else 0)
            self.d2meta = ("dgrad2_1x1<bf16,C64>", self.out.npix * 64 * nops * esz)
            P.note_launch(self.d2meta[0], self.d2meta[1], 2.0 * self.out.npix * 128 * self.out.C)
        if self.wdesc is not None:
            w, wg = self.wdesc, self.wgeom
            ctn = -(-w.Cout // 16)
            ctn = 4 if ctn == 3 else (8 if ctn > 4 else ctn)
            nkw = -(-(wg.kext // 16) // 4)
            nkw = 1 if nkw <= 1 else 2 if nkw <= 2 else 3 if nkw <= 3 else 5 if nkw <= 5 else 10
            if wg.lean == 2:
                self.wkey = f"rowwgrad_kernel<{T},C{wg.cch},CO{w.Cout},K{w.KH}>"
            elif wg.lean:
                self.wkey = f"wgrad_lean_kernel<{T},C{wg.cch},CO{w.Cout},K{w.KH}>"
            else:
                self.wkey = f"wgrad_kernel<{T},CT{ctn},NK{nkw}>"
            self.wbytes = (w.B * w.Hin * w.Win * (w.C1 + w.C2) * wg.nchunks // wg.nchunks + w.B * w.Hout * w.Wout * w.Cout) * esz \
                + w.nslabs * wg.slab_bytes
            if not self.wg_fused:
                P.note_launch(self.wkey, self.wbytes, self.flops)
            if self.kind != "conv":
                P.note_launch("msau_channel_sum", self.out.npix * self.out.Cs * esz, 0.0)

    def fwd(self, s):
        if self.pair is not None and self.pair.active:
            if self is self.pair.c2:
                L.call("msau_conv_pair", s, self.plan.dtype, C.byref(self.pair.fdesc), key=self.pair.key)
            return
        if self.cpl_fused_into is not None:
            return
        L.call("msau_conv2d", s, self.plan.dtype, C.byref(self.fdesc), key=self.fkey)

    def fwd_recs(self):
        rm = self.plan.rec_meta
        if self.cpl_fused_into is not None:
            return []
        if self.pair is not None and self.pair.active:
            if self is not self.pair.c2:
                return []
            rm[C.addressof(self.pair.fdesc)] = (self.pair.key, self.pair.fbytes)
            return [(L.OP_CONV_PAIR, self.pair.fdesc)]
        rm[C.addressof(self.fdesc)] = (self.fkey, self.fbytes)
        return [(L.OP_CONV2D, self.fdesc)]

    def bwd_recs(self):
        if self.wdesc is None:
            return []
        side = L.OP_SIDE if self.plan.overlap_wgrad else 0
        if self.x1 is self.plan.x_in:
            side = 0
        recs = [] if self.wg_fused else [(L.OP_WGRAD | side, self.wdesc)]
        if self.kind != "conv":
            P = self.plan
            self._csum = L.CsumArgs(_ptr(self.out.grad), self.out.npix, self.out.Cs, P.slab_ptr(self.csum_off), self.csum_blocks)
            recs.append((L.OP_CHANNEL_SUM | side, self._csum))
        rm = self.plan.rec_meta
        if not self.wg_fused:
            rm[C.addressof(self.wdesc)] = (self.wkey, self.wbytes)
        if self.pair is not None and self.pair.active and self.pair.bdesc is not None:
            if self is self.pair.c2:
                rm[C.addressof(self.pair.bdesc)] = (self.pair.key, self.pair.bbytes)
                if self.pair.dcp is not None:
                    return [(L.OP_CONV_PAIR, self.pair.bdesc)] + recs
                recs.append((L.OP_CONV_PAIR, self.pair.bdesc))
            return recs
        if self.dgrad_in_pair is not None:
            return recs
        if self.proj is not None and self.proj.active:
            return recs + (self.proj.recs() if self is self.proj.f else [])
        if self.dgrad2 is not None:
            rm[C.addressof(self.dgrad2)] = self.d2meta
            return recs + [(L.OP_DGRAD2_1X1, self.dgrad2)]
        for si, dd in enumerate(self.ddesc):
            if dd is not None:
                rm[C.addressof(dd)] = self.dmeta[si]
                recs.append((L.OP_CONV2D, dd))
        return recs

    def bwd_wgrad(self, s):
        if self.wdesc is None or self.wg_fused:
            return
        P = self.plan
        L.call("msau_conv2d_wgrad", s, P.dtype, C.byref(self.wdesc), key=self.wkey)
        if self.kind != "conv":
            L.call("msau_channel_sum", s, P.dtype, _ptr(self.out.grad), self.out.npix, self.out.Cs,
                   P.slab_ptr(self.csum_off), self.csum_blocks)

    def bwd_dgrad(self, s):
        if self.wdesc is None:
            return
        P = self.plan
        if self.pair is not None and self.pair.active and self.pair.bdesc is not None:
            if self is self.pair.c2:
                L.call("msau_conv_pair", s, P.dtype, C.byref(self.pair.bdesc), key=self.pair.key)
            return
        if self.proj is not None and self.proj.active:
            if self is self.proj.f:
                self.proj.launch(s)
            return
        if self.dgrad2 is not None:
            L.call("msau_dgrad2_1x1", s, P.dtype, C.byref(self.dgrad2), key=self.d2meta[0])
            return
        if self.dgrad_in_pair is not None:
            return
        for si, dd in enumerate(self.ddesc):
            if dd is not None:
                L.call("msau_conv2d", s, P.dtype, C.byref(dd), key=self.dmeta[si][0])

    def bwd(self, s):
        if self.pair is not None and self.pair.active and self.pair.dcp is not None and self is self.pair.c2:
            self.bwd_dgrad(s)
            self.bwd_wgrad(s)
            return
        self.bwd_wgrad(s)
        self.bwd_dgrad(s)


class PairOp:

    def __init__(self, plan: "Plan", c1: ConvOp, c2: ConvOp):
        self.plan, self.c1, self.c2 = plan, c1, c2
        self.active = False
        self.fdesc = self.bdesc = None
        self.dcp: Optional[ConvOp] = None
        c1.pair = c2.pair = self
        plan.pairs.append(self)

    def bind(self):
        P, c1, c2 = self.plan, self.c1, self.c2
        x0, r1, out = c1.x1, c1.out, c2.out
        if os.environ.get("MSAU_FUSE_PAIR", "1") == "0" or not P.cfg.get("fuse_pair", True) or P.generic_only:
            return
        ok = (c1.kind == c2.kind == "conv" and c1.k == c2.k == 3 and c1.dil == c2.dil == 1 and c1.x2 is None and c2.x2 is None
              and c1.relu_in and c1.relu_out and c1.fwd_add is None and not c2.relu_in and c2.relu_out and c2.fwd_add is x0
              and c2.x1 is r1 and x0.C == x0.Cs == r1.C == out.C and x0.Cs in (8, 16, 32) and not c1.head and not c2.head
              and r1.n_contrib == (1 if P.training else 0))
        if not ok:
            return
        f = L.ConvPairDesc()
        f.B, f.H, f.W, f.C = P.B, x0.H, x0.W, x0.Cs
        f.flags1, f.flags2 = L.PAIR_RELU_IN | L.PAIR_RELU_MID, L.CONV_ADD | L.CONV_RELU_OUT
        f.x, f.w1, f.b1, f.mid = _ptr(x0.data), P.pack_ptr(c1.w_off), P.pack_ptr(c1.b_off), _ptr(r1.data)
        f.w2, f.b2, f.add, f.y = P.pack_ptr(c2.w_off), P.pack_ptr(c2.b_off), _ptr(x0.data), _ptr(out.data)
        if not L.load().msau_conv_pair_applicable(P.dtype, C.byref(f)):
            return
        pool = getattr(c2, "pool", None)
        if pool is not None and x0.Cs < int(os.environ.get("MSAU_PAIR_POOL_MINC", "16")):
            pool.fused_into = None
            pool = None
        if pool is not None:
            f.flags2 |= L.CONV_POOL
            f.pool_y, f.pool_idx = _ptr(pool.y.data), _ptr(pool.idx)
            if L.load().msau_conv_pair_applicable(P.dtype, C.byref(f)):
                pool.fused_into = self
            else:
                f.flags2 &= ~L.CONV_POOL
                pool.fused_into = None
        self.fdesc = f
        T = "f32" if P.dtype == L.F32 else "bf16"
        esz = 4 if P.dtype == L.F32 else 2
        self.key = f"conv_pair_kernel<{T},C{x0.Cs}>"
        n = P.B * x0.H * x0.W * x0.Cs
        self.fbytes = 3 * n * esz
        if f.flags2 & L.CONV_POOL:
            self.fbytes += (n // 4) * (esz + 1)
        if P.training and c1.ddesc[0] is not None and c2.ddesc[0] is not None and c1.ddesc[1] is None and c2.ddesc[1] is None \
                and c1.d_off[0] is not None and c2.d_off[0] is not None:
            d1, d2 = c1.ddesc[0], c2.ddesc[0]
            if d2.flags == L.CONV_MASK_B and not (d1.flags & ~(L.CONV_MASK_A | L.CONV_ADD | L.CONV_ACCUM | L.CONV_MASK_B)):
                b = L.ConvPairDesc()
                b.B, b.H, b.W, b.C = P.B, x0.H, x0.W, x0.Cs
                b.flags1, b.flags2 = L.PAIR_MASK_MID, d1.flags
                b.x, b.w1, b.b1, b.mask_mid, b.mid = _ptr(out.grad), P.pack_ptr(c2.d_off[0]), None, d2.mask_b, _ptr(r1.grad)
                b.w2, b.b2, b.add, b.mask_a, b.mask_b, b.y = P.pack_ptr(c1.d_off[0]), None, d1.add, d1.mask_a, d1.mask_b, d1.y
                use_bits = os.environ.get("MSAU_PAIR_BITS", "1") != "0"
                if use_bits:
                    b.bits_mid = b.bits_a = 1
                if L.load().msau_conv_pair_applicable(P.dtype, C.byref(b)):
                    self.bdesc = b
                else:
                    b.bits_mid = b.bits_a = None
                self.bbytes = 5 * n * esz
                if self.bdesc is not None and use_bits:
                    nbits = int(L.load().msau_conv_pair_bits_bytes(P.dtype, C.byref(b)))
                    if nbits != int(L.load().msau_conv_pair_bits_bytes(P.dtype, C.byref(f))):
                        f.flags1 |= L.PAIR_TILES
# ... 185 lines not shown

    def bwd(self, s):
        if self.ws is not None:
            L.call("msau_box_bwd", s, self.plan.dtype, C.byref(self._ba), key=self.bkey)

    def load_params(self, s, flat_params: torch.Tensor):
        a = self._fa
        L.call("msau_box_params", s, flat_params.data_ptr(), a.off_hmin, a.off_hmax, a.off_wmin, a.off_wmax, a.C, a.F, a.max_h, a.max_w,
               self.params[0].data_ptr(), self.params[1].data_ptr())


class LrnOp(Op):

    def __init__(self, plan, name, a: Act, y: Act):
        self.plan, self.name, self.a, self.y = plan, name, a, y
        self.slot = a.register() if a.needs_grad else None
        self.stage = plan._cur_stage
        self.fused_into = None
        self.bwd_fused_into = None
        y.lrn_producer = self
        prod = plan.ops[-1] if plan.ops else None
        if isinstance(prod, ConvOp) and prod.out is a and os.environ.get("MSAU_FUSE_LRN", "1") != "0":
            prod.lrn = self
        plan.ops.append(self)

    def reads(self):
        return [self.a]

    def writes(self):
        return [self.y]

    def note(self):
        P, a = self.plan, self.a
        esz = 4 if P.dtype == L.F32 else 2
        T = "f32" if P.dtype == L.F32 else "bf16"
        n = a.npix * a.Cs * esz
        self.fkey, self.bkey = f"lrn_fwd<{T},C{a.Cs}>", f"lrn_bwd<{T},C{a.Cs}>"
        self.fbytes, self.bbytes = 2 * n, 3 * n
        if self.fused_into is None:
            P.note_launch(self.fkey, self.fbytes, 0.0)
        if P.training and self.y.grad is not None and a.grad is not None and self.bwd_fused_into is None:
            P.note_launch(self.bkey, self.bbytes, 0.0)

    def fwd_recs(self):
        a, y = self.a, self.y
        if self.fused_into is not None:
            return []
        self._fa = L.LrnArgs(_ptr(a.data), None, _ptr(y.data), a.npix, a.C, a.Cs, a.C, 1e-4, 0.75, 1.0)
        self.plan.rec_meta[C.addressof(self._fa)] = (self.fkey, self.fbytes)
        return [(L.OP_LRN_FWD, self._fa)]

    def bwd_recs(self):
        a, y = self.a, self.y
        if y.grad is None or a.grad is None or self.bwd_fused_into is not None:
            return []
        self._ba = L.LrnArgs(_ptr(a.data), _ptr(y.grad), _ptr(a.grad), a.npix, a.C, a.Cs, a.C, 1e-4, 0.75, 1.0)
        self.plan.rec_meta[C.addressof(self._ba)] = (self.bkey, self.bbytes)
        return [(L.OP_LRN_BWD, self._ba)]

    def fwd(self, s):
        a, y = self.a, self.y
        if self.fused_into is not None:
            return
        L.call("msau_lrn_fwd", s, self.plan.dtype, _ptr(a.data), _ptr(y.data), a.npix, a.C, a.Cs, a.C, 1e-4, 0.75, 1.0, key=self.fkey)

    def bwd(self, s):
        a, y = self.a, self.y
        if y.grad is None or a.grad is None or self.bwd_fused_into is not None:
            return
        assert a.n_contrib == 1 and not a.relu_out
        L.call("msau_lrn_bwd", s, self.plan.dtype, _ptr(a.data), _ptr(y.grad), _ptr(a.grad), a.npix, a.C, a.Cs, a.C,
               1e-4, 0.75, 1.0, key=self.bkey)


class PoolOp(Op):

    def __init__(self, plan, name, x: Act, y: Act):
        self.plan, self.name, self.x, self.y = plan, name, x, y
        assert y.H == (x.H + 1) // 2 and y.W == (x.W + 1) // 2 and y.Cs == x.Cs
        self.idx = torch.zeros((plan.B, y.H, y.W, y.Cs), dtype=torch.uint8, device=plan.device) if plan.training else None
        self.slot = x.register() if x.needs_grad else None
        self.stage = plan._cur_stage
        self.fused_into = None
        prod = plan.ops[-1] if plan.ops else None
        if isinstance(prod, ConvOp) and prod.out is x and os.environ.get("MSAU_FUSE_POOL", "1") != "0":
            prod.pool = self
        plan.ops.append(self)

    def reads(self):
        return [self.x]

    def writes(self):
        return [self.y]

    def note(self):
        P, x, y = self.plan, self.x, self.y
        esz = 4 if P.dtype == L.F32 else 2
        T = "f32" if P.dtype == L.F32 else "bf16"
        nx, ny = x.npix * x.Cs, y.npix * y.Cs
        self.fkey, self.bkey = f"pool_fwd<{T},C{x.Cs}>", f"pool_bwd<{T},C{x.Cs}>"
        self.fbytes = (nx + ny) * esz + (ny if P.training else 0)
        if self.fused_into is None:
            P.note_launch(self.fkey, self.fbytes, 0.0)
        self.bbytes = 0
        if P.training and y.grad is not None and x.grad is not None:
            accum, maskb = x.slot_flags(self.slot)
            self.bbytes = (ny + nx * (1 + int(accum) + int(maskb))) * esz + ny
            P.note_launch(self.bkey, self.bbytes, 0.0)

    def fwd_recs(self):
        x, y = self.x, self.y
        if self.fused_into is not None:
            return []
        self._fa = L.PoolArgs(_ptr(x.data), _ptr(y.data), _ptr(self.idx), None, self.plan.B, x.H, x.W, x.Cs, 0, None)
        self.plan.rec_meta[C.addressof(self._fa)] = (self.fkey, self.fbytes)
        return [(L.OP_POOL_FWD, self._fa)]

    def bwd_recs(self):
        x, y = self.x, self.y
        if y.grad is None or x.grad is None:
            return []
        accum, maskb = x.slot_flags(self.slot)
        self._ba = L.PoolArgs(_ptr(y.grad), _ptr(x.grad), _ptr(self.idx), _ptr(x.data) if maskb else None,
                              self.plan.B, x.H, x.W, x.Cs, int(accum) | (2 if maskb and self.plan.act_flag else 0),
                              self.plan.extent_ptr(x))
        self.plan.rec_meta[C.addressof(self._ba)] = (self.bkey, self.bbytes)
        return [(L.OP_POOL_BWD, self._ba)]

    def fwd(self, s):
        x, y = self.x, self.y
        if self.fused_into is not None:
            return
        L.call("msau_maxpool2x2_fwd", s, self.plan.dtype, _ptr(x.data), _ptr(y.data), _ptr(self.idx), self.plan.B, x.H, x.W, x.Cs,
               key=self.fkey)

    def bwd(self, s):
        x, y = self.x, self.y
        if y.grad is None or x.grad is None:
            return
        accum, maskb = x.slot_flags(self.slot)
        L.call("msau_maxpool2x2_bwd_ext", s, self.plan.dtype, _ptr(y.grad), _ptr(self.idx), _ptr(x.grad),
               _ptr(x.data) if maskb else None, self.plan.B, x.H, x.W, x.Cs, int(accum) | (2 if maskb and self.plan.act_flag else 0),
               self.plan.extent_ptr(x), key=self.bkey)


class AttnCoreOp(Op):

    def __init__(self, plan, name, f: Act, g: Act, h: Act, x: Act, y: Act):
        self.plan, self.name, self.f, self.g, self.h, self.x, self.y = plan, name, f, g, h, x, y
        self.N = x.H * x.W
        self.stats = torch.zeros((plan.B, self.N, 2), dtype=torch.float32, device=plan.device)
        self.ws = torch.zeros((plan.B, self.N), dtype=torch.float32, device=plan.device)
        for t in (f, g, h):
            t.register()
        self.stage = plan._cur_stage
        plan.ops.append(self)

    def reads(self):
        return [self.f, self.g, self.h, self.x]

    def writes(self):
        return [self.y]

    def _args(self, bwd):
        return L.AttnArgs(_ptr(self.f.data), _ptr(self.g.data), _ptr(self.h.data),
                          _ptr(self.y.grad) if bwd else _ptr(self.x.data), _ptr(self.y.data), _ptr(self.stats),
                          _ptr(self.f.grad), _ptr(self.g.grad), _ptr(self.h.grad), _ptr(self.ws),
                          self.plan.B, self.N, self.f.Cs, self.h.Cs, self.plan.extent_ptr(self.x), self.x.W)

    def note(self):
        P = self.plan
        esz = 4 if P.dtype == L.F32 else 2
        T = "f32" if P.dtype == L.F32 else "bf16"
        npx = P.B * self.N
        small, big = npx * self.f.Cs * esz, npx * self.h.Cs * esz
        self.fkey, self.bkey = f"selfattn_fwd<{T}>", f"selfattn_bwd<{T}>"
        self.fbytes = 2 * small + 3 * big
        ffl = 2.0 * P.B * self.N * self.N * (self.f.C + self.h.C)
        P.note_launch(self.fkey, self.fbytes, ffl)
        self.bbytes = 4 * small + 4 * big
        if P.training and self.y.grad is not None:
            P.note_launch(self.bkey, self.bbytes, 2.0 * ffl)

    def fwd_recs(self):
        self._fa = self._args(False)
        self.plan.rec_meta[C.addressof(self._fa)] = (self.fkey, self.fbytes)
        return [(L.OP_ATTN_FWD, self._fa)]

    def bwd_recs(self):
        if self.y.grad is None:
            return []
        self._ba = self._args(True)
        self.plan.rec_meta[C.addressof(self._ba)] = (self.bkey, self.bbytes)
        return [(L.OP_ATTN_BWD, self._ba)]

    def fwd(self, s):
        L.call("msau_selfattn_fwd_ext", s, self.plan.dtype, _ptr(self.f.data), _ptr(self.g.data), _ptr(self.h.data),
               _ptr(self.x.data), _ptr(self.y.data), _ptr(self.stats), self.plan.B, self.N, self.f.Cs, self.h.Cs,
               self.plan.extent_ptr(self.x), self.x.W, key=self.fkey)

    def bwd(self, s):
        if self.y.grad is None:
            return
        L.call("msau_selfattn_bwd_ext", s, self.plan.dtype, _ptr(self.f.data), _ptr(self.g.data), _ptr(self.h.data),
               _ptr(self.y.grad), _ptr(self.stats), _ptr(self.f.grad), _ptr(self.g.grad), _ptr(self.h.grad),
               _ptr(self.ws), self.plan.B, self.N, self.f.Cs, self.h.Cs, self.plan.extent_ptr(self.x), self.x.W, key=self.bkey)


class ProjBwd:

    def __init__(self, plan: "Plan", f: ConvOp, g: ConvOp, h: ConvOp):
        self.plan, self.f, self.g, self.h = plan, f, g, h
        self.active = False
        self.args = None
        for c in (f, g, h):
            c.proj = self
        plan.projs.append(self)

    def bind(self):
        P, f, g, h = self.plan, self.f, self.g, self.h
        x = f.x1
# ... 277 lines not shown
        self.ext_slot = {}
        if self.training:
            for t in (self.logits, self.aux):
                if t is not None:
                    self.ext_slot[t.name] = t.register()
        if self.reuse:
            self._assign_buffers()
        if not self.training and self.logits.C <= 255:
            lg = self.logits
            self.head_probs = torch.zeros((self.B, lg.H, lg.W, lg.C), dtype=torch.float32, device=self.device)
            self.head_argmax = torch.zeros((self.B, lg.H, lg.W), dtype=torch.uint8, device=self.device)
        for a in self.acts:
            a.alloc_grad()
        for op in self.ops:
            op.finalize()
        if self.box_ops:
            self.box_ii_g = torch.zeros((max(self.box_scratch, 1),), dtype=torch.float32, device=self.device)
            self.box_ws = torch.zeros((max(self.box_ws_ii, 1),), dtype=torch.float32, device=self.device)
        self.pack_arena = torch.zeros(max(self._pack_bytes, 256), dtype=torch.uint8, device=self.device)
        for op in self.ops:
            if isinstance(op, ConvOp):
                op.bind()
        for pr in self.pairs:
            pr.bind()
        for pj in self.projs:
            pj.bind()
        self.slab_arena = torch.zeros(max(self._slab_elems, 64), dtype=torch.float32, device=self.device)
        for op in self.ops:
            if isinstance(op, ConvOp):
                op.late_bind()
        for pj in self.projs:
            pj.late_bind()
        for pr in self.pairs:
            pr.late_bind()
            pr.note()
        for op in self.ops:
            if not isinstance(op, ConvOp):
                op.note()
        self._note_boundary()
        side_ops, join_ops = set(), set()
        if self.training and self.overlap_wgrad and os.environ.get("MSAU_ATTN_SIDE", "1") != "0":
            for op in self.ops:
                if isinstance(op, AttnCoreOp):
                    branch = [c for c in self.ops if isinstance(c, ConvOp) and c.out in (op.f, op.g, op.h)]
                    users = [c for c in self.ops if c is not op and any(t is op.y for t in c.reads())]
                    later = self.ops[self.ops.index(op) + 1:]
                    first = min(users, key=self.ops.index) if users else None
                    if len(branch) == 3 and users and all(u in later for u in users) and \
                            isinstance(first, ConvOp) and first.fwd_recs() and \
                            not any(t in (op.f, op.g, op.h) for o2 in later for t in o2.reads()):
                        side_ops.update(id(c) for c in branch)
                        side_ops.add(id(op))
                        join_ops.add(id(first))
        frecs = []
        for op in self.ops:
            for kind, args in op.fwd_recs():
                if id(op) in side_ops:
                    kind |= L.OP_SIDE
                elif id(op) in join_ops:
                    kind |= L.OP_JOIN
                    join_ops.discard(id(op))
                frecs.append((kind, args))
        assert not join_ops, "a side-stream attention branch lost its join: its first reader emitted no launch record"
        self._fwd_side = bool(side_ops)

        self._fwd_seq = self._make_seq(frecs)
        self.pack_table = self._upload(self._pack_entries, L.PackEntry) if self._pack_entries else None
        self.unpack_table = self._upload(self._unpack_entries, L.UnpackEntry) if self._unpack_entries else None
        self._bwd_seq, self._bwd_segs, self._reduce_args = None, [], []
        if self.training:
            recs = []
            stages = sorted({op.stage for op in self.ops}, reverse=True)
            esz = C.sizeof(L.UnpackEntry)
            def reduce_rec(group):
                idx = [i for i, st in enumerate(self._unpack_stage) if st == group]
                if not idx:
                    return
                assert idx == list(range(idx[0], idx[-1] + 1)), "unpack entries of a group must be contiguous"
                ra = L.ReduceArgs(self.slab_arena.data_ptr(), None, self.unpack_table.data_ptr() + idx[0] * esz,
                                  len(idx), self._unpack_max)
                self._reduce_args.append(ra)
                recs.append((L.OP_WGRAD_REDUCE | (L.OP_SIDE if self.overlap_wgrad else 0), ra))

            for b in stages:
                start = len(recs)
                ops_b = [op for op in reversed(self.ops) if op.stage == b]
                cut = next((i for i, op in enumerate(ops_b) if isinstance(op, ConvOp) and op.reduce_group() != b), len(ops_b))
                assert all(not isinstance(op, ConvOp) or op.reduce_group() != b for op in ops_b[cut:]), \
                    "separately reduced convs must close their stage's backward"
                recs += [r for op in ops_b[:cut] for r in op.bwd_recs()]
                reduce_rec(b)
                if cut < len(ops_b):
                    recs += [r for op in ops_b[cut:] for r in op.bwd_recs()]
                    reduce_rec(-1)
                self._bwd_segs.append((b, start, len(recs) - start))
            self._bwd_seq = self._make_seq(recs)
        HW = self.H * self.W
        lg = self.logits
        self.out_logits = torch.zeros((self.B, lg.C, lg.H, lg.W), dtype=torch.float32, device=self.device)
        self.out_aux = torch.zeros((self.B, self.aux.C, self.aux.H, self.aux.W), dtype=torch.float32,
                                   device=self.device) if self.aux is not None else None
        if self.training:
            self.counts_k = max(1, min(16, 256 // self.B)) if self.B <= 1024 and os.environ.get("MSAU_LABEL_SPLIT", "1") != "0" else 1
            self.counts = torch.zeros((self.B * self.counts_k,), dtype=torch.int32, device=self.device)
            self.ce_ws = torch.zeros((int(L.load().msau_ce_ws_floats(self.B * HW)),), dtype=torch.float32, device=self.device)
            self.ce_multi_ws = torch.zeros((int(L.load().msau_ce_multi_ws_floats(self.B * HW)),), dtype=torch.float32, device=self.device)
            self.loss_buf = torch.zeros((1,), dtype=torch.float32, device=self.device)

    def _assign_buffers(self):
        last_read: Dict[int, int] = {}
        for i, op in enumerate(self.ops):
            for t in op.reads():
                last_read[id(t)] = i
        keep = {id(t) for t in getattr(self, "stage_logits", [])} | {id(t) for t in (self.logits, self.aux) if t is not None}
        free: Dict[int, List[torch.Tensor]] = {}
        self.buffers: List[torch.Tensor] = []

        def take(a: Act):
            n = self.B * a.H * a.W * a.Cs
            pool = free.setdefault(n, [])
            if pool:
                buf = pool.pop()
            else:
                buf = torch.zeros((n,), dtype=self.tdtype, device=self.device)
                self.buffers.append(buf)
            a.data = buf.view(self.B, a.H, a.W, a.Cs)
            a._buf = buf

        def release(a: Act):
            if id(a) not in keep and a.data is not None:
                free[a._buf.numel()].append(a._buf)

        take(self.x_in)
        for i, op in enumerate(self.ops):
            for t in op.writes():
                if t.data is None:
                    take(t)
            for t in set(op.reads()) | set(op.writes()):
                if last_read.get(id(t), -1) <= i and (t in op.reads() or id(t) not in last_read):
                    release(t)
        for a in self.acts:
            if a.data is None:
                take(a)

    def _note_boundary(self):
        esz = 4 if self.dtype == L.F32 else 2
        a = self.x_in
        self.in_bytes = self.B * a.C * a.H * a.W * 4 + a.npix * a.Cs * esz
        c = self._nchw_first_conv()
        if c is None:
            self.note_launch("msau_nchw_to_nhwc", self.in_bytes, 0.0)
        else:
            self.unnote_launch(c.fkey, c.fbytes, c.flops)
            T = "f32" if self.dtype == L.F32 else "bf16"
            c.fkey = f"first_conv_nchw<{T},CIN{a.Cs},CO{c.out.Cs}>"
            c.fbytes = self.B * a.C * a.H * a.W * 4 + (a.npix * a.Cs * esz if self.training else 0) + c.out.npix * c.out.Cs * esz
            self.note_launch(c.fkey, c.fbytes, c.flops)
        nparam = sum(int(math.prod(shp)) for shp in self.pshape.values())
        self.note_launch("msau_pack_params", nparam * 4 + self._pack_bytes, 0.0)
        if self.training:
            HW = self.H * self.W
            lg = self.logits
            nl = 2 if self.aux is not None else 1
            self.note_launch("msau_label_counts", self.B * HW * 8, 0.0)
            self.ce_bytes = self.B * HW * (8 + nl * 2 * lg.Cs * esz)
            self.note_launch("msau_masked_ce_multi" if lg.Cs <= 16 else "msau_masked_ce", self.ce_bytes, 0.0)
            self.reduce_bytes = self._slab_elems * 4 + nparam * 4
            self.note_launch("msau_wgrad_reduce", self.reduce_bytes, 0.0)
            self.note_launch("msau_clip_adam_step", nparam * 4 * 8, 0.0)

    def set_probe_keys(self, keys, side: bool = False) -> List[Tuple[str, float]]:
        order = []
        for seq in (self._fwd_seq, self._bwd_seq):
            if seq is None:
                continue
            arr, cnt, _ = seq
            for i in range(cnt):
                meta = self.rec_meta.get(arr[i].args)
                if keys is not None and meta is not None and meta[0] in keys and bool(arr[i].kind & L.OP_SIDE) == side:
                    arr[i].kind |= L.OP_PROBE
                    order.append(meta)
                else:
                    arr[i].kind &= ~L.OP_PROBE
        return order

    def set_probe(self, key: Optional[str]) -> int:
        want = set()
        if key is not None:
            for op in self.ops:
                if isinstance(op, ConvOp):
                    if op.fkey == key:
                        want.add(C.addressof(op.fdesc))
                    for si, dd in enumerate(op.ddesc):
                        if dd is not None and op.dmeta[si][0] == key:
                            want.add(C.addressof(dd))
            for pr in self.pairs:
                if pr.active and pr.key == key:
                    want.add(C.addressof(pr.fdesc))
                    if pr.bdesc is not None:
                        want.add(C.addressof(pr.bdesc))
        n = 0
        for seq in (self._fwd_seq, self._bwd_seq):
            if seq is None:
                continue
            arr, cnt, _ = seq
            for i in range(cnt):
                if arr[i].args in want:
                    arr[i].kind |= L.OP_PROBE
                    n += 1
                else:
                    arr[i].kind &= ~L.OP_PROBE
        return n

    @staticmethod
    def read_probe(cap: int = 1 << 16):
        buf = (C.c_float * cap)()
        n = C.c_int(0)
        L.call("msau_probe_read", buf, cap, C.byref(n))
        return list(buf[:n.value])

    def _make_seq(self, recs):
        arr = (L.Op * max(len(recs), 1))()
        for i, (kind, args) in enumerate(recs):
            arr[i].kind, arr[i].dtype, arr[i].args = kind, self.dtype, C.addressof(args)
        return arr, len(recs), recs

    def _run_seq(self, seq, s):
        L.call("msau_run_ops", s, seq[0], seq[1])

    def _upload(self, entries, ctype):
        n = len(entries)
        arr = (ctype * n)(*entries)
        raw = bytes(memoryview(arr))
        host = torch.frombuffer(bytearray(raw), dtype=torch.uint8)
        return host.to(self.device)

    @staticmethod
    def _stream() -> int:
        return torch.cuda.current_stream().cuda_stream

    def pack(self, flat_params: torch.Tensor):
        if self.pack_table is None:
            return
        L.call("msau_pack_params", self._stream(), flat_params.data_ptr(), self.pack_arena.data_ptr(),
               self.pack_table.data_ptr(), len(self._pack_entries), self._pack_max)
        for bop in self.box_ops:
            bop.load_params(self._stream(), flat_params)

    def load_input(self, x_nchw: torch.Tensor):
        assert x_nchw.dtype == torch.float32 and x_nchw.is_contiguous() and tuple(x_nchw.shape) == \
            (self.B, self.cfg["channels"], self.H, self.W), (x_nchw.shape, x_nchw.dtype)
        a = self.x_in
        L.call("msau_nchw_to_nhwc", self._stream(), self.dtype, x_nchw.data_ptr(), a.data.data_ptr(), self.B, a.C, a.Cs, self.H, self.W)
        if self.ragged:
            self._zero_outside(a.data, a.data, 1, self.H, self.W, a.data.element_size() * a.Cs)

    def _nchw_first_conv(self):
        if not hasattr(self, "_nchw_conv"):
            c = next((op for op in self.ops if isinstance(op, ConvOp) and op.x1 is self.x_in and op.x2 is None), None)
            ok = c is not None and os.environ.get("MSAU_FIRST_NCHW", "1") != "0" and not (c.pair is not None and c.pair.active) \
                and not (c.fdesc.flags & ~L.CONV_RELU_OUT)
            if ok:
                info = (L.i32 * 8)()
                L.call("msau_conv2d_launch_info", self.dtype, C.byref(c.fdesc), info)
                ok = bool(info[7] & 64)
            self._nchw_conv = c if ok else None
            self._nchw_on = False
        return self._nchw_conv

    def _feed_nchw(self, x_nchw: Optional[torch.Tensor]) -> bool:
        c = self._nchw_first_conv()
        if c is None:
            return False
        if x_nchw is not None:
            assert x_nchw.dtype == torch.float32 and x_nchw.is_contiguous() and tuple(x_nchw.shape) == \
                (self.B, self.cfg["channels"], self.H, self.W), (x_nchw.shape, x_nchw.dtype)
            if x_nchw.data_ptr() % 16:
                x_nchw = None
# ... 335 lines not shown
```

Measured before the change: 5722 tiles/s.

## Fuse maxpool backward scatter into the preceding conv's dgrad epilogue

Adds a new lean-conv epilogue (EPI_POOL_BWD) that takes the dgrad output tile held in registers and scatters it through the 2x2 maxpool argmax indices straight into the pool input's gradient, with optional accumulate and mask. The plan binds this op for convs whose input is a pool output, skips the separate maxpool backward launch, and checks record ordering. The aim is to remove a kernel launch and the write-then-reread of the pooled gradient. Only two specific dilated bf16 conv shapes qualify, and the added epilogue work and launch-bounds hint could raise register pressure.

```diff
diff --git a/include/msau_hip.h b/include/msau_hip.h
--- a/include/msau_hip.h
+++ b/include/msau_hip.h
@@ -89,6 +89,17 @@
                             int stride, int ups, msau_conv_pack_geom* out);
 int msau_conv2d(void* stream, int dtype, const msau_conv_desc* d);
 int msau_conv2d_launch_info(int dtype, const msau_conv_desc* d, int32_t* info8);
+
+typedef struct {
+    msau_conv_desc conv;
+    void* dx;
+    const uint8_t* idx;
+    const void* mask;
+    int32_t H, W;
+    int32_t accumulate;
+    int32_t reserved;
+} msau_conv_pool_bwd_args;
+int msau_conv2d_pool_bwd(void* stream, int dtype, const msau_conv_pool_bwd_args* a);
 
 enum { MSAU_PAIR_RELU_IN = 1, MSAU_PAIR_RELU_MID = 2, MSAU_PAIR_MASK_MID = 4,
        MSAU_PAIR_LRN_BWD = 16,
@@ -324,7 +335,8 @@
     MSAU_OP_BOX_BWD = 13,
     MSAU_OP_ALLREDUCE = 14,
     MSAU_OP_ATTN_PROJ_BWD = 15,
-    MSAU_OP_DGRAD2_1X1 = 16
+    MSAU_OP_DGRAD2_1X1 = 16,
+    MSAU_OP_CONV_POOL_BWD = 17
 };
 typedef struct { int32_t kind; int32_t dtype; const void* args; } msau_op;
 typedef struct { const void* a; const void* dy; void* out; int64_t npix; int32_t C, Cs, n; float alpha, beta, k; } msau_lrn_args;
diff --git a/msau_amd/_lib.py b/msau_amd/_lib.py
--- a/msau_amd/_lib.py
+++ b/msau_amd/_lib.py
@@ -116,6 +116,11 @@
 class Dgrad2Args(C.Structure):
     _fields_ = [(n, vp) for n in ("g", "w1_pack", "w2_pack", "dx1", "dx2", "mask1", "mask2")] + \
                [("npix", i64), ("C", i32), ("accumulate1", i32), ("accumulate2", i32), ("reserved", i32)]
+
+
+class ConvPoolBwdArgs(C.Structure):
+    _fields_ = [("conv", ConvDesc), ("dx", vp), ("idx", vp), ("mask", vp), ("H", i32), ("W", i32), ("accumulate", i32),
+                ("reserved", i32)]
 
 
 OP_SIDE = 0x100
@@ -128,6 +133,7 @@
 OP_BOX_FWD, OP_BOX_BWD = 12, 13
 OP_ATTN_PROJ_BWD = 15
 OP_DGRAD2_1X1 = 16
+OP_CONV_POOL_BWD = 17
 OP_CONV2D, OP_WGRAD, OP_LRN_FWD, OP_LRN_BWD, OP_POOL_FWD, OP_POOL_BWD, OP_ATTN_FWD, OP_ATTN_BWD, OP_CHANNEL_SUM = range(1, 10)
 
 _SIGNATURES = {
@@ -142,6 +148,7 @@
     "msau_conv2d_rider_slabs": (C.c_int, [C.c_int, C.POINTER(ConvDesc)]),
     "msau_attn_proj_bwd": (C.c_int, [vp, C.c_int, C.POINTER(AttnProjBwdArgs)]),
     "msau_dgrad2_1x1": (C.c_int, [vp, C.c_int, C.POINTER(Dgrad2Args)]),
+    "msau_conv2d_pool_bwd": (C.c_int, [vp, C.c_int, C.POINTER(ConvPoolBwdArgs)]),
     "msau_conv2d_launch_info": (C.c_int, [C.c_int, C.POINTER(ConvDesc), C.POINTER(i32)]),
     "msau_conv_pair_applicable": (C.c_int, [C.c_int, C.POINTER(ConvPairDesc)]),
     "msau_conv_pair": (C.c_int, [vp, C.c_int, C.POINTER(ConvPairDesc)]),
@@ -217,7 +224,7 @@
 EXPORTED_SYMBOLS = tuple(_SIGNATURES)
 
 ABI_STRUCTS = (ConvDesc, WgradDesc, PackEntry, UnpackEntry, Op, LrnArgs, PoolArgs, AttnArgs, CsumArgs, ReduceArgs,
-               ConvPackGeom, WgradGeom, ConvPairDesc, BoxArgs, AllreduceArgs, OwnerCtx, AttnProjBwdArgs, Dgrad2Args)
+               ConvPackGeom, WgradGeom, ConvPairDesc, BoxArgs, AllreduceArgs, OwnerCtx, AttnProjBwdArgs, Dgrad2Args, ConvPoolBwdArgs)
 
 
 class MsauHipError(RuntimeError):
diff --git a/msau_amd/csrc/conv.hip b/msau_amd/csrc/conv.hip
--- a/msau_amd/csrc/conv.hip
+++ b/msau_amd/csrc/conv.hip
@@ -329,6 +329,10 @@
 int msau_conv_lean_ids_capable(int dtype, const msau_conv_desc* d, int nchunks, int CT);
 int msau_conv_chunked_try(hipStream_t s, int dtype, const msau_conv_desc* d, int cch, int kchunk, int nchunks, int CT);
 int msau_conv_chunked_capable(int dtype, const msau_conv_desc* d, int cch, int nchunks, int CT);
+int msau_conv_pool_bwd_capable(int dtype, const msau_conv_desc* d, int cch, int nchunks, int CT);
+int msau_conv_pool_bwd_try(hipStream_t s, int dtype, const msau_conv_desc* d, void* dx, const uint8_t* idx, const void* mask, int H, int W,
+                           int accumulate, int cch, int kchunk, int nchunks, int CT);
+static int conv_takes_pool_bwd(int dtype, const msau_conv_desc* d);
 int msau_firstconv_takes(int dtype, const msau_conv_desc* d);
 int msau_firstconv_launch(hipStream_t s, int dtype, const msau_conv_desc* d, int real_channels);
 
@@ -371,6 +375,7 @@
         p.flags |= MSAU_CONV_EXTENT;
         if (conv_takes_extent(dtype, &p, g)) info[7] |= 128;
     }
+    if (conv_takes_pool_bwd(dtype, d)) info[7] |= 256;
     if (g.nslices == 1 && !(info[7] & 4)) {
         msau_conv_desc p = *d;
         p.flags |= MSAU_CONV_LRN;
@@ -501,3 +506,33 @@
     }
     return 0;
 }
+
+static int conv_takes_pool_bwd(int dtype, const msau_conv_desc* d) {
+    ConvGeom g;
+    if (conv_geom(dtype, d->C1, d->C2, d->Cout, d->KH, d->KW, d->dil, d->stride, d->ups, &g)) return 0;
+    if (g.nslices != 1 || msau_rowconv_takes(dtype, d)) return 0;
+    return msau_conv_pool_bwd_capable(dtype, d, g.cch, g.nchunks, g.CT);
+}
+
+extern "C" int msau_conv2d_pool_bwd(void* stream, int dtype, const msau_conv_pool_bwd_args* a) {
+    MSAU_CHECK_ARG(a && a->conv.x1 && a->conv.wpack && a->conv.y && a->dx && a->idx, "conv2d_pool_bwd: null pointer");
+    const msau_conv_desc* d = &a->conv;
+    MSAU_CHECK_ARG(d->B > 0 && d->Hout > 0 && d->Wout > 0 && a->H > 0 && a->W > 0 && (a->H + 1) / 2 == d->Hout &&
+                   (a->W + 1) / 2 == d->Wout && d->Cout % 8 == 0 && (a->accumulate == 0 || a->accumulate == 1),
+                   "conv2d_pool_bwd: the pool input is H x W = %d x %d, the launch's output %d x %d (must be ceil(H/2) x ceil(W/2))",
+                   a->H, a->W, d->Hout, d->Wout);
+    MSAU_CHECK_ARG((int64_t)a->H * a->W * d->Cout * (dtype == MSAU_F32 ? 4 : 2) < (1ll << 31), "conv2d_pool_bwd: image too large");
+    MSAU_CHECK_ARG(!(d->flags & MSAU_CONV_ADD) || d->add, "conv2d_pool_bwd: ADD without pointer");
+    MSAU_CHECK_ARG(!(d->flags & MSAU_CONV_MASK_A) || d->mask_a, "conv2d_pool_bwd: MASK_A without pointer");
+    MSAU_CHECK_ARG(!(d->flags & MSAU_CONV_MASK_B) || d->mask_b, "conv2d_pool_bwd: MASK_B without pointer");
+    if (!conv_takes_pool_bwd(dtype, d))
+        return msau_set_error(MSAU_ERR_ARG, "conv2d_pool_bwd: no instance with the pool-backward epilogue takes this launch (flags 0x%x; see "
+                              "msau_conv2d_launch_info info[7] & 256); run msau_conv2d, then msau_maxpool2x2_bwd", d->flags);
+    ConvGeom g;
+    int rc = conv_geom(dtype, d->C1, d->C2, d->Cout, d->KH, d->KW, d->dil, d->stride, d->ups, &g);
+    if (rc) return rc;
+    rc = msau_conv_pool_bwd_try(static_cast<hipStream_t>(stream), dtype, d, a->dx, a->idx, a->mask, a->H, a->W, a->accumulate,
+                                g.cch, g.kchunk, g.nchunks, g.CT);
+    if (rc == 0) return msau_set_error(MSAU_ERR_ARG, "conv2d_pool_bwd: the launch was not taken");
+    return rc < 0 ? rc : 0;
+}
diff --git a/msau_amd/csrc/conv_lean.hip b/msau_amd/csrc/conv_lean.hip
--- a/msau_amd/csrc/conv_lean.hip
+++ b/msau_amd/csrc/conv_lean.hip
@@ -2,6 +2,13 @@
 #include <cstdlib>
 
 namespace {
+
+struct PoolBwdOps {
+    void* dx;
+    const uint8_t* idx;
+    const void* mask;
+    int H, W, accumulate;
+};
 
 struct LeanArgs {
     msau_conv_desc d;
@@ -12,6 +19,7 @@
     unsigned mag_tx, mag_ty;
     int per_xcd;
     int ct_total;
+    PoolBwdOps pb;
 #ifdef MSAU_STAMPS
     unsigned long long* stamps;
 #endif
@@ -43,10 +51,62 @@
 };
 
 constexpr int kOperandBits = MSAU_CONV_RELU_IN | MSAU_CONV_RELU_OUT | MSAU_CONV_ADD | MSAU_CONV_ACCUM | MSAU_CONV_MASK_A | MSAU_CONV_MASK_B;
-enum { EPI_NONE = 0, EPI_LRN = 1, EPI_POOL = 2, EPI_HEAD = 3 };
+enum { EPI_NONE = 0, EPI_LRN = 1, EPI_POOL = 2, EPI_HEAD = 3, EPI_POOL_BWD = 4 };
+
+template <typename T, int RG, int NWR>
+__device__ __forceinline__ void pool_bwd_rows(const PoolBwdOps& pb, const typename Vec4<T>::type (&g)[4], int b, int oy0, int ox, int ch,
+                                              int wr0, int Ho, int Wo, int Cs) {
+    typedef typename Vec4<T>::type V4;
+    constexpr int ESZ = (int)sizeof(T), NP = 2 * NWR;
+    const long long img = (long long)pb.H * pb.W * Cs * ESZ;
+    char* dxb = static_cast<char*>(pb.dx) + b * img;
+    const char* mb = pb.mask ? static_cast<const char*>(pb.mask) + b * img : nullptr;
+    const uint8_t* ib = pb.idx + (long long)b * Ho * Wo * Cs;
+    const unsigned prow = (unsigned)pb.W * Cs * ESZ;
+#pragma unroll
+    for (int p0 = 0; p0 < 4; p0 += RG) {
+        V4 old[RG][NP], m[RG][NP];
+        unsigned packed[RG];
+#pragma unroll
+        for (int r = 0; r < RG; ++r) {
+            const int oy = oy0 + p0 + r;
+            if (oy >= Ho) continue;
+            packed[r] = *reinterpret_cast<const unsigned*>(ib + ((unsigned)oy * Wo + ox) * Cs + ch);
+            const unsigned o = (2u * oy + wr0) * prow + ((unsigned)(2 * ox) * Cs + ch) * ESZ;
+#pragma unroll
+            for (int q = 0; q < NP; ++q) {
+                const bool ok = 2 * oy + wr0 + (q >> 1) < pb.H && 2 * ox + (q & 1) < pb.W;
+                const unsigned op = o + (q >> 1) * prow + (q & 1) * Cs * ESZ;
+#pragma unroll
+                for (int j = 0; j < 4; ++j) old[r][q][j] = (T)0.f;
+                if (pb.accumulate && ok) old[r][q] = *reinterpret_cast<const V4*>(dxb + op);
+                if (mb && ok) m[r][q] = *reinterpret_cast<const V4*>(mb + op);
+            }
+        }
+#pragma unroll
+        for (int r = 0; r < RG; ++r) {
+            const int oy = oy0 + p0 + r;
+            if (oy >= Ho) continue;
+            const unsigned o = (2u * oy + wr0) * prow + ((unsigned)(2 * ox) * Cs + ch) * ESZ;
+#pragma unroll
+            for (int q = 0; q < NP; ++q) {
+                if (!(2 * oy + wr0 + (q >> 1) < pb.H && 2 * ox + (q & 1) < pb.W)) continue;
+                const int pos = 2 * wr0 + q;
+                V4 v4;
+#pragma unroll
+                for (int j = 0; j < 4; ++j) {
+                    float v = (float)old[r][q][j] + ((int)((packed[r] >> (8 * j)) & 0xff) == pos ? (float)g[p0 + r][j] : 0.f);
+                    if (mb && !((float)m[r][q][j] > 0.f)) v = 0.f;
+                    v4[j] = (T)v;
+                }
+                *reinterpret_cast<V4*>(dxb + o + (q >> 1) * prow + (q & 1) * Cs * ESZ) = v4;
+            }
+        }
+    }
+}
 template <typename T, int CIN8, int CT, int KS, bool DUAL, int DIL = 1, int WGW = 1, bool DOUT = false, bool SPLIT = false,
           int STRIDE = 1, int UPS = 1, int EPI = EPI_NONE, int EOP = -1, bool IDS = false>
-__global__ __launch_bounds__(256 * WGW) void conv_lean_kernel(const LeanArgs a) {
+__global__ __launch_bounds__(256 * WGW, EPI == EPI_POOL_BWD && CIN8 <= 2 ? 4 : 1) void conv_lean_kernel(const LeanArgs a) {
     static_assert(!IDS || (!DUAL && STRIDE == 1 && UPS == 1 && !DOUT && !SPLIT), "id-mask input: plain single-source instances");
     static_assert(!SPLIT || (CT == 1 && !DUAL && !DOUT && WGW == 1), "SPLIT instances are single-source, one tile per workgroup");
     static_assert((STRIDE == 1 && UPS == 1) || (!DUAL && !DOUT && WGW == 1 && DIL == 1 && STRIDE * UPS == 2), "strided / upsampling instances");
@@ -298,10 +358,10 @@
                 }
             }
         } else {
-        constexpr bool POOL_OK = EPI == EPI_POOL;
+        constexpr bool POOL_OK = EPI == EPI_POOL, KEEP = POOL_OK || EPI == EPI_POOL_BWD;
         static_assert(EPI == EPI_NONE || (CT <= 2 && !DOUT && STRIDE == 1 && UPS == 1), "fused epilogues: <= 2 channel tiles, one output");
-        V4 keep[POOL_OK ? CT : 1][4];
-        if constexpr (POOL_OK) {
+        V4 keep[KEEP ? CT : 1][4];
+        if constexpr (KEEP) {
 #pragma unroll
             for (int ct = 0; ct < CT; ++ct)
 #pragma unroll
@@ -349,8 +409,30 @@
 #pragma unroll
                         for (int j = 0; j < 4; ++j) o[j] = (T)v[j];
                         *reinterpret_cast<V4*>(yp) = o;
-                        if constexpr (POOL_OK) keep[ct][pt] = o;
-                    }
+                        if constexpr (KEEP) keep[ct][pt] = o;
+                    }
+                }
+            }
+        }
+        if constexpr (EPI == EPI_POOL_BWD) {
+            static_assert(!SPLIT && !DUAL, "pool backward: all channels of the pooled pixel from one workgroup, one source");
+            const int col = ox0 + cwt * 16 + lr;
+            if constexpr (CT == 1 && CIN8 == 2) {
+                V4 g[4];
+#pragma unroll
+                for (int pt = 0; pt < 4; ++pt) {
+                    typedef int dwords __attribute__((ext_vector_type(2)));
+                    dwords src = __builtin_bit_cast(dwords, keep[0][pt]), dst;
+#pragma unroll
+                    for (int w = 0; w < 2; ++w) dst[w] = __shfl_xor(src[w], 32);
+                    g[pt] = lg >= 2 ? __builtin_bit_cast(V4, dst) : keep[0][pt];
+                }
+                if (col < d.Wout) pool_bwd_rows<T, 2, 1>(a.pb, g, b, oyw, col, (lg & 1) * 4, lg >> 1, d.Hout, d.Wout, Cout);
+            } else if (col < d.Wout) {
+#pragma unroll
+                for (int ct = 0; ct < CT; ++ct) {
+                    const int ch = lg * (CTT * 4) + (cty + ct) * 4;
+                    if (ch < Cout) pool_bwd_rows<T, 4, 2>(a.pb, keep[ct], b, oyw, col, ch, 0, d.Hout, d.Wout, Cout);
                 }
             }
         }
@@ -961,3 +1043,41 @@
     if (dtype == MSAU_F32) return d->KH == 3 ? lean_cin<float, 3>(s, a, cin8, dual, CT) : lean_cin<float, 1>(s, a, cin8, dual, CT);
     return d->KH == 3 ? lean_cin<bf16_t, 3>(s, a, cin8, dual, CT) : lean_cin<bf16_t, 1>(s, a, cin8, dual, CT);
 }
+
+static int pool_bwd_case(int dtype, const msau_conv_desc* d, int cch, int nchunks, int CT) {
+    if (dtype != MSAU_BF16 || d->C2 || d->KH != 3 || d->KW != 3 || d->stride != 1 || d->ups != 1) return 0;
+    if (d->flags) return 0;
+    if (chunked_variant(dtype, d, cch, nchunks, CT) || !msau_conv_lean_applicable(dtype, d, nchunks, CT) || lean_split_wanted(d, CT)) return 0;
+    if (d->dil == 4 && d->C1 == 32 && d->Cout == 16 && CT == 1) return 2;
+    if (d->dil == 2 && d->C1 == 16 && d->Cout == 8 && CT == 1) return 3;
+    return 0;
+}
+int msau_conv_pool_bwd_capable(int dtype, const msau_conv_desc* d, int cch, int nchunks, int CT) {
+    return pool_bwd_case(dtype, d, cch, nchunks, CT) != 0;
+}
+int msau_conv_pool_bwd_try(hipStream_t s, int dtype, const msau_conv_desc* d, void* dx, const uint8_t* idx, const void* mask, int H, int W,
+                           int accumulate, int cch, int kchunk, int nchunks, int CT) {
+    const int which = pool_bwd_case(dtype, d, cch, nchunks, CT);
+    if (!which) return 0;
+    LeanArgs a;
+    a.d = *d;
+    a.kchunk = kchunk;
+    a.in_px1 = d->C1 * 2; a.in_row1 = d->Win * a.in_px1; a.in_px2 = a.in_row2 = 0;
+    a.out_px = d->Cout * 2; a.out_row = d->Wout * a.out_px;
+    a.tiles_x = cdiv(d->Wout, 16); a.tiles_y = cdiv(d->Hout, 16);
+    a.ntiles = d->B * a.tiles_x * a.tiles_y;
+    if (a.ntiles >= (1 << 20) || a.tiles_x >= 4096 || a.tiles_y >= 4096) return 0;
+    a.mag_tx = (unsigned)((0x100000000ull + a.tiles_x - 1) / a.tiles_x);
+    a.mag_ty = (unsigned)((0x100000000ull + a.tiles_y - 1) / a.tiles_y);
+    a.per_xcd = 0; a.ct_total = CT;
+    a.pb.dx = dx; a.pb.idx = idx; a.pb.mask = mask;
+    a.pb.H = H; a.pb.W = W; a.pb.accumulate = accumulate;
+#ifdef MSAU_STAMPS
+    a.stamps = nullptr;
+#endif
+    switch (which) {
+        case 2: return launch_lean_e<bf16_t, 4, 1, 3, false, 4, 1, false, false, 1, 1, EPI_POOL_BWD, 0>(s, a);
+        case 3: return launch_lean_e<bf16_t, 2, 1, 3, false, 2, 1, false, false, 1, 1, EPI_POOL_BWD, 0>(s, a);
+        default: return 0;
+    }
+}
diff --git a/msau_amd/csrc/pack.hip b/msau_amd/csrc/pack.hip
--- a/msau_amd/csrc/pack.hip
+++ b/msau_amd/csrc/pack.hip
@@ -37,6 +37,7 @@
         case 15: return (int)sizeof(msau_owner_ctx);
         case 16: return (int)sizeof(msau_attn_proj_bwd_args);
         case 17: return (int)sizeof(msau_dgrad2_args);
+        case 18: return (int)sizeof(msau_conv_pool_bwd_args);
         default: return -1;
     }
 }
diff --git a/msau_amd/csrc/sequence.hip b/msau_amd/csrc/sequence.hip
--- a/msau_amd/csrc/sequence.hip
+++ b/msau_amd/csrc/sequence.hip
@@ -214,6 +214,7 @@
             case MSAU_OP_BOX_BWD: rc = msau_box_bwd(stream, o.dtype, static_cast<const msau_box_args*>(o.args)); break;
             case MSAU_OP_ATTN_PROJ_BWD: rc = msau_attn_proj_bwd(stream, o.dtype, static_cast<const msau_attn_proj_bwd_args*>(o.args)); break;
             case MSAU_OP_DGRAD2_1X1: rc = msau_dgrad2_1x1(stream, o.dtype, static_cast<const msau_dgrad2_args*>(o.args)); break;
+            case MSAU_OP_CONV_POOL_BWD: rc = msau_conv2d_pool_bwd(stream, o.dtype, static_cast<const msau_conv_pool_bwd_args*>(o.args)); break;
             case MSAU_OP_LRN_FWD: {
                 const msau_lrn_args* a = static_cast<const msau_lrn_args*>(o.args);
                 rc = msau_lrn_fwd(stream, o.dtype, a->a, a->out, a->npix, a->C, a->Cs, a->n, a->alpha, a->beta, a->k);
diff --git a/msau_amd/plan.py b/msau_amd/plan.py
--- a/msau_amd/plan.py
+++ b/msau_amd/plan.py
@@ -114,6 +114,9 @@
         for x in (x1, x2):
             self.slots.append(x.register() if (x is not None and x.needs_grad) else None)
         self.stage = plan._cur_stage
+        prev = plan.ops[-1] if plan.ops else None
+        self.pool_src = prev if isinstance(prev, PoolOp) and prev.y is x1 and x2 is None and kind == "conv" else None
+        self.pbargs = None
         plan.ops.append(self)
 
     def reduce_group(self):
@@ -385,12 +388,34 @@
                 dd.flags &= ~L.CONV_WGRAD
                 dd.wg_x1 = dd.wg_slabs = None
 
+    def _bind_pool_bwd(self):
+        P, pl, dd = self.plan, self.pool_src, self.ddesc[0]
+        if pl is None or dd is None or os.environ.get("MSAU_FUSE_POOL_BWD", "1") == "0" or P.generic_only or P.act_flag:
+            return
+        x = pl.x
+        if x.grad is None or pl.y.grad is None or self.slots[0] != 0 or self.ddesc[1] is not None or self.dd_off is not None \
+                or self.dgrad2 is not None or self.dgrad_in_pair is not None or (self.proj is not None and self.proj.active) \
+                or (self.pair is not None and self.pair.active):
+            return
+        info = (L.i32 * 8)()
+        L.call("msau_conv2d_launch_info", P.dtype, C.byref(dd), info)
+        if not info[7] & 256:
+            return
+        accum, maskb = x.slot_flags(pl.slot)
+        a = L.ConvPoolBwdArgs()
+        a.conv = dd
+        a.dx, a.idx, a.mask = _ptr(x.grad), _ptr(pl.idx), (_ptr(x.data) if maskb else None)
+        a.H, a.W, a.accumulate = x.H, x.W, int(accum)
+        self.pbargs = a
+        pl.bwd_fused_into = self
+
     def late_bind(self):
         P = self.plan
         if self.wdesc is not None:
             self.wdesc.slabs = P.slab_ptr(self.slab_off)
         if self.wg_fused and self.pair is None and self.ddesc[0] is not None and self.ddesc[0].flags & L.CONV_WGRAD:
             self.ddesc[0].wg_slabs = P.slab_ptr(self.wg_slab_off)
+        self._bind_pool_bwd()
         T = "f32" if P.dtype == L.F32 else "bf16"
         esz = 4 if P.dtype == L.F32 else 2
         taps = self.k * self.k
@@ -431,6 +456,11 @@
                 src_c = (self.x1.C + self.x2.C) if self.dd_off is not None else (self.x1, self.x2)[si].C
                 fl = 2.0 * P.B * (self.out.H * self.out.W if self.kind == "conv" else self.x1.H * self.x1.W) * taps * src_c * self.out.C
                 self.dmeta[si] = conv_meta(dd)
+                if si == 0 and self.pbargs is not None:
+                    a, px = self.pbargs, self.pool_src.x
+                    name, nb = self.dmeta[0]
+                    nb += px.npix * px.Cs * (1 + a.accumulate + (1 if a.mask else 0)) * esz + self.x1.npix * self.x1.Cs
+                    self.dmeta[0] = (name[:-1] + ",pool_bwd>", nb)
                 if (self.proj is None or not self.proj.active) and self.dgrad2 is None and self.dgrad_in_pair is None:
                     P.note_launch(self.dmeta[si][0], self.dmeta[si][1], fl)
         if self.dgrad2 is not None:
@@ -506,6 +536,9 @@
         if self.dgrad2 is not None:
             rm[C.addressof(self.dgrad2)] = self.d2meta
             return recs + [(L.OP_DGRAD2_1X1, self.dgrad2)]
+        if self.pbargs is not None:
+            rm[C.addressof(self.pbargs)] = self.dmeta[0]
+            return recs + [(L.OP_CONV_POOL_BWD, self.pbargs)]
         for si, dd in enumerate(self.ddesc):
             if dd is not None:
                 rm[C.addressof(dd)] = self.dmeta[si]
@@ -537,6 +570,9 @@
             L.call("msau_dgrad2_1x1", s, P.dtype, C.byref(self.dgrad2), key=self.d2meta[0])
             return
         if self.dgrad_in_pair is not None:
+            return
+        if self.pbargs is not None:
+            L.call("msau_conv2d_pool_bwd", s, P.dtype, C.byref(self.pbargs), key=self.dmeta[0][0])
             return
         for si, dd in enumerate(self.ddesc):
             if dd is not None:
@@ -888,6 +924,7 @@
         self.slot = x.register() if x.needs_grad else None
         self.stage = plan._cur_stage
         self.fused_into = None
+        self.bwd_fused_into = None
         prod = plan.ops[-1] if plan.ops else None
         if isinstance(prod, ConvOp) and prod.out is x and os.environ.get("MSAU_FUSE_POOL", "1") != "0":
             prod.pool = self
@@ -909,7 +946,7 @@
         if self.fused_into is None:
             P.note_launch(self.fkey, self.fbytes, 0.0)
         self.bbytes = 0
-        if P.training and y.grad is not None and x.grad is not None:
+        if P.training and y.grad is not None and x.grad is not None and self.bwd_fused_into is None:
             accum, maskb = x.slot_flags(self.slot)
             self.bbytes = (ny + nx * (1 + int(accum) + int(maskb))) * esz + ny
             P.note_launch(self.bkey, self.bbytes, 0.0)
@@ -924,7 +961,7 @@
 
     def bwd_recs(self):
         x, y = self.x, self.y
-        if y.grad is None or x.grad is None:
+        if y.grad is None or x.grad is None or self.bwd_fused_into is not None:
             return []
         accum, maskb = x.slot_flags(self.slot)
         self._ba = L.PoolArgs(_ptr(y.grad), _ptr(x.grad), _ptr(self.idx), _ptr(x.data) if maskb else None,
@@ -942,7 +979,7 @@
 
     def bwd(self, s):
         x, y = self.x, self.y
-        if y.grad is None or x.grad is None:
+        if y.grad is None or x.grad is None or self.bwd_fused_into is not None:
             return
         accum, maskb = x.slot_flags(self.slot)
         L.call("msau_maxpool2x2_bwd_ext", s, self.plan.dtype, _ptr(y.grad), _ptr(self.idx), _ptr(x.grad),
@@ -1386,18 +1423,33 @@
                 self._reduce_args.append(ra)
                 recs.append((L.OP_WGRAD_REDUCE | (L.OP_SIDE if self.overlap_wgrad else 0), ra))
 
+            span = {}
+
+            def op_recs(ops):
+                for op in ops:
+                    i0 = len(recs)
+                    recs.extend(op.bwd_recs())
+                    span[id(op)] = (i0, len(recs))
+
             for b in stages:
                 start = len(recs)
                 ops_b = [op for op in reversed(self.ops) if op.stage == b]
                 cut = next((i for i, op in enumerate(ops_b) if isinstance(op, ConvOp) and op.reduce_group() != b), len(ops_b))
                 assert all(not isinstance(op, ConvOp) or op.reduce_group() != b for op in ops_b[cut:]), \
                     "separately reduced convs must close their stage's backward"
-                recs += [r for op in ops_b[:cut] for r in op.bwd_recs()]
+                op_recs(ops_b[:cut])
                 reduce_rec(b)
                 if cut < len(ops_b):
-                    recs += [r for op in ops_b[cut:] for r in op.bwd_recs()]
+                    op_recs(ops_b[cut:])
                     reduce_rec(-1)
                 self._bwd_segs.append((b, start, len(recs) - start))
+            for pl in self.ops:
+                if isinstance(pl, PoolOp) and pl.bwd_fused_into is not None:
+                    fused = span[id(pl.bwd_fused_into)]
+                    assert span[id(pl)][0] == span[id(pl)][1] and recs[fused[1] - 1][1] is pl.bwd_fused_into.pbargs
+                    for op in self.ops:
+                        if op is not pl and pl.x in op.writes() and span[id(op)][0] < span[id(op)][1]:
+                            assert span[id(op)][0] >= fused[1], f"{op.name}: backward record ahead of the launch that finishes {pl.x.name}.grad"
             self._bwd_seq = self._make_seq(recs)
         HW = self.H * self.W
         lg = self.logits
@@ -1498,6 +1550,8 @@
                     for si, dd in enumerate(op.ddesc):
                         if dd is not None and op.dmeta[si][0] == key:
                             want.add(C.addressof(dd))
+                            if si == 0 and op.pbargs is not None:
+                                want.add(C.addressof(op.pbargs))
             for pr in self.pairs:
                 if pr.active and pr.key == key:
                     want.add(C.addressof(pr.fdesc))
```

Result: no change. 5746 tiles/s, median of 6 (+0.4%).
